# kostas1515/object_detectors

Hardware: AMD Instinct MI355X
Metric: images/sec (fwd+bwd) YOLOv3 640px bs=32 (higher is better)
Workload: dtype bf16; 1 GPU; YOLOv3 Darknet-53 training step (fwd+loss+bwd+SGD step), synthetic COCO 640px, per-GPU bs=32, 7 GT/img, random-init weights; global_batch=32, parallelism=dp1

## Files before the change

### include/mi355det.h

```cpp
#ifndef MI355DET_H
#define MI355DET_H

#include <stddef.h>
#include <stdint.h>

#ifdef __cplusplus
extern "C" {
#endif

#define MI355DET_OK 0
#define MI355DET_EINVAL (-1)
#define MI355DET_ELAUNCH (-2)
#define MI355DET_EWORKSPACE (-3)

#define MI355DET_MAX_SCALES 4
#define MI355DET_MAX_ANCHORS 8

const char* mi355det_last_error(void);
int mi355det_debug_set(int key, int value);
int mi355det_debug_ptr(int key, void* ptr);
int mi355det_version(void);

typedef struct {
  int32_t num_scales, na, num_classes, pad0;
// ... 94 lines not shown
                        float wy, float ww, float wh, float* rois, int64_t* out_labels, int64_t* out_matched, float* out_regression_targets,
                        void* stream);

int mi355det_match_anchors(const float* gt, const float* anchors, int32_t m, int64_t n, float high_thr,
                           float low_thr, int allow_low_quality, uint32_t* gt_best, int64_t* matches,
                           void* stream);

int mi355det_box_encode(const float* reference_boxes, const float* proposals, float* out, int64_t n,
                        float wx, float wy, float ww, float wh, void* stream);
int mi355det_box_decode(const float* codes, const float* boxes, float* out, int64_t n, int32_t k,
                        float wx, float wy, float ww, float wh, float clip, void* stream);

int mi355det_anchor_grid(const float* cell, int32_t a, int32_t gh, int32_t gw, int32_t stride_h,
                         int32_t stride_w, float* out, void* stream);

int mi355det_sigmoid_focal_loss(const float* x, const float* t, const float* scale, const uint8_t* valid,
                                int64_t rows, int32_t k, float alpha, float gamma, float grad_scale,
                                float* loss_sum, float* grad, void* stream);
int mi355det_sigmoid_focal_loss_elem(const float* x, const float* t, int64_t n, float alpha, float gamma, float* loss,
                                     float* grad, void* stream);

int mi355det_retina_cls_loss(const float* logits, const int64_t* matched, const int64_t* gt_labels,
                             const float* scale, int64_t rows, int32_t k, float alpha, float gamma,
                             float grad_scale, float* loss_sum, float* grad, void* stream);

int mi355det_retina_loss(const float* cls_logits, const float* bbox_regression, const float* anchors, const int64_t* matched,
                         const float* gt_boxes, const int64_t* gt_labels, const int32_t* gt_offsets,
                         const float* class_scale, int32_t n_images, int64_t rows_per_image, int32_t k, float alpha,
                         float gamma, float grad_scale, float* num_fg, float* losses, float* grad_logits,
                         float* grad_regression, void* stream);

typedef struct {
  int32_t n_levels;
  int32_t anchors_per_pixel;
  int64_t pixels[8];
  void* grad[8];
  int32_t grad_ld[8];
} mi355det_level_grads;
int mi355det_retina_loss_lv(const float* cls_logits, const float* bbox_regression, const float* anchors, const int64_t* matched,
                            const float* gt_boxes, const int64_t* gt_labels, const int32_t* gt_offsets, const float* class_scale,
                            int32_t n_images, int64_t rows_per_image, int32_t k, float alpha, float gamma, float grad_scale,
                            float* num_fg, float* losses, const mi355det_level_grads* cls_levels, float* grad_regression, void* stream);

int mi355det_roi_align(const float* const* feats, const int32_t* hs, const int32_t* ws, const float* scales,
                       int32_t num_levels, const float* rois, int32_t num_rois, int32_t channels,
                       int32_t pooled_h, int32_t pooled_w, int32_t sampling_ratio, int aligned, int32_t k_min,
                       int32_t k_max, float* out, const float* grad_out, float* const* grad_feats, void* stream);

int mi355det_roi_align_nhwc(const void* const* feats, const int32_t* hs, const int32_t* ws, const int32_t* lds,
                            const float* scales, int32_t num_levels, const float* rois, int32_t num_rois,
                            int32_t channels, int32_t pooled_h, int32_t pooled_w, int32_t sampling_ratio, int aligned,
                            int32_t k_min, int32_t k_max, float* out, const float* grad_out, float* const* grad_feats,
                            void* stream);

int mi355det_topk(const float* x, int32_t rows, int64_t n, int64_t row_stride, int32_t k, float min_value,
                  int64_t* idx_out, float* val_out, int32_t* count_out, void* stream);
size_t mi355det_topk_workspace(int32_t rows);
int mi355det_topk_ws(const float* x, int32_t rows, int64_t n, int64_t row_stride, int32_t k, float min_value, int64_t* idx_out,
                     float* val_out, int32_t* count_out, void* workspace, size_t workspace_bytes, void* stream);

int mi355det_topk_segments(const float* x, int32_t rows, int64_t row_stride, int32_t nseg, const int64_t* seg_start, const int64_t* seg_n,
                           const int32_t* seg_k, float min_value, int64_t* const* idx_out, float* const* val_out, int32_t* const* count_out,
                           void* workspace, size_t workspace_bytes, void* stream);

typedef struct {
  int32_t n, h, w, cin;
  int32_t ho, wo, cout;
  int32_t ksize, stride, pad;
  int32_t in_ld, out_ld;
} mi355det_conv_shape;

int mi355det_conv_fwd(const mi355det_conv_shape* s, const void* x, const void* w, const float* bias,
                      void* y, int out_f32, float* stats, int32_t cout_pad, void* stream);
typedef struct {
  const float* scale;
  const float* shift;
  const void* residual;
  int32_t residual_ld;
  int32_t relu;
  int64_t out_image_stride;
  float slope;
} mi355det_conv_epilogue;
int mi355det_conv_fwd_ex(const mi355det_conv_shape* s, const void* x, const void* w, const mi355det_conv_epilogue* e,
                         void* y, int out_f32, int32_t cout_pad, void* stream);
int mi355det_conv_autotune_mode(int on);

typedef struct {
  uint32_t table;
  int32_t value;
  uint64_t key;
} mi355det_tune_entry;
size_t mi355det_tune_export(void* buf, size_t cap);
int mi355det_tune_import(const void* buf, size_t bytes, int replace);
int mi355det_tune_lock(int on);
int mi355det_tune_clear(void);
int mi355det_conv_stats_rows(const mi355det_conv_shape* s, int32_t cout_pad);
int mi355det_stem_im2col(const float* img, void* out, int32_t n, int32_t h, int32_t w, void* stream);

int mi355det_stem_l1_rows(int32_t n, int32_t h, int32_t w);
int mi355det_stem_l1_fwd(const float* img, const void* w0, const float* scale_shift0, float slope, const void* w1, void* a0,
                         int32_t a0_ld, void* z1, int32_t z1_ld, float* stats, int32_t n, int32_t h, int32_t w, void* stream);
int mi355det_stem_l1_fwd_eval(const float* img, const void* w0, const float* scale_shift0, float slope, const void* w1,
                              const float* scale_shift1, void* a1, int32_t a1_ld, int32_t n, int32_t h, int32_t w, void* stream);
int mi355det_stem_rows(int32_t n, int32_t h, int32_t w);
int mi355det_stem_fwd_stats(const float* img, const void* w, float* partial, int32_t n, int32_t h, int32_t wd, void* stream);
int mi355det_stem_fwd_apply(const float* img, const void* w, const float* scale_shift, float slope, void* a, int32_t a_ld,
                            int32_t n, int32_t h, int32_t wd, void* stream);
int mi355det_stem_bwd_reduce(const float* img, const void* w, const float* scale_shift, float slope, const void* da,
                             int32_t da_ld, float* partial, int32_t n, int32_t h, int32_t wd, void* stream);
int mi355det_stem_bwd_apply_wgrad(const float* img, const void* w, const float* scale_shift, const float* sums, float slope,
                                  const void* da, int32_t da_ld, float* slab, float* dw, float* dgamma, float* dbeta,
                                  int32_t n, int32_t h, int32_t wd, void* stream);

int mi355det_stem_bwd_fused(const float* img, const void* w, const float* scale_shift, float slope, const void* da, int32_t da_ld,
                            float* slab, float* ag, float* sums, int32_t n, int32_t h, int32_t wd, void* stream);
int mi355det_stem_bwd_finish(const void* w, const float* scale_shift, const float* ag, const float* sums, int64_t count, float* dw,
                             float* dgamma, float* dbeta, void* stream);

int mi355det_conv_dgrad(const mi355det_conv_shape* s, const void* dy, const void* wt, void* dx,
                        const void* residual, int32_t residual_ld, void* stream);

int mi355det_conv_dgrad_mask(const mi355det_conv_shape* s, const void* dy, const void* wt, void* dx, const void* act, int32_t act_ld,
                             const float* scale, int32_t relu, void* stream);
size_t mi355det_conv_dgrad_workspace(const mi355det_conv_shape* s);
int mi355det_conv_dgrad_ws(const mi355det_conv_shape* s, const void* dy, const void* wt, void* dx, const void* residual, int32_t residual_ld,
                           void* workspace, size_t workspace_bytes, void* stream);

int mi355det_conv_dgrad_bn_rows(const mi355det_conv_shape* s);
int mi355det_conv_dgrad_bn(const mi355det_conv_shape* s, const void* dy, const void* wt, void* dx, const void* residual,
                           int32_t residual_ld, const void* z, int32_t z_ld, const float* scale_shift, float slope,
                           float* partials, void* stream);
int mi355det_bn_bwd_sum_partials(const float* partials, int32_t rows, int32_t c, int32_t c_pad, float* sums,
                                 void* stream);

size_t mi355det_conv_wgrad_workspace(const mi355det_conv_shape* s);
int mi355det_conv_wgrad_autotune(const mi355det_conv_shape* s, const void* x, const void* dy, float* dw,
                                 void* workspace, size_t workspace_bytes, void* stream);
int mi355det_conv_wgrad(const mi355det_conv_shape* s, const void* x, const void* dy, float* dw,
                        float* dbias, void* workspace, size_t workspace_bytes, void* stream);

size_t mi355det_dgrad_pack_elems(const mi355det_conv_shape* s);
int mi355det_pack_weights(const mi355det_conv_shape* s, const float* w, int w_is_ohwi, void* w_fwd,
                          int32_t cout_pad, void* w_dgrad, void* stream);
typedef struct {
  const float* w;
  void* w_fwd;
  void* w_dgrad;
  mi355det_conv_shape shape;
  int32_t cout_pad, w_is_ohwi;
} mi355det_pack_item;
size_t mi355det_pack_table_bytes(const mi355det_pack_item* items, int32_t n, int32_t* n_entries, int32_t* n_blocks);
int mi355det_pack_table_build(const mi355det_pack_item* items, int32_t n, void* host_table, size_t host_bytes);
int mi355det_pack_weights_batched(const void* dev_table, int32_t n_entries, int32_t n_blocks, void* stream);
int mi355det_unpack_wgrad(const mi355det_conv_shape* s, const float* dw, float* grad, void* stream);

size_t mi355det_gconv_pack_elems(const mi355det_conv_shape* s, int32_t groups);
int mi355det_gconv_pack_weights(const mi355det_conv_shape* s, int32_t groups, const float* w, int w_is_ohwi, void* w_fwd, void* w_dgrad,
                                void* stream);
int mi355det_gconv_fwd_ex(const mi355det_conv_shape* s, int32_t groups, const void* x, const void* w_fwd, const mi355det_conv_epilogue* e,
                          void* y, int out_f32, void* stream);
int mi355det_gconv_dgrad(const mi355det_conv_shape* s, int32_t groups, const void* dy, const void* w_dgrad, void* dx, void* stream);
size_t mi355det_gconv_wgrad_workspace(const mi355det_conv_shape* s, int32_t groups);
int mi355det_gconv_wgrad(const mi355det_conv_shape* s, int32_t groups, const void* x, const void* dy, float* dw, void* workspace,
                         size_t workspace_bytes, void* stream);

int mi355det_bn_finalize(const float* stats, int32_t rows, int32_t c, int32_t c_pad, int64_t count,
                         const float* gamma, const float* beta, float eps, float momentum,
                         float* running_mean, float* running_var,
                         float* scale_shift , void* stream);
int mi355det_bn_fold_partials_f64(const float* stats, int32_t rows, int32_t c, int32_t c_pad, double* sums64, void* stream);
int mi355det_bn_finalize_f64(const double* sums64, int32_t c, int32_t c_pad, int64_t count, const float* gamma, const float* beta,
                             float eps, float momentum, float* running_mean, float* running_var, float* scale_shift,
                             void* stream);
int mi355det_bn_eval_scale_shift(int32_t c, const float* gamma, const float* beta, const float* running_mean,
                                 const float* running_var, float eps, float* scale_shift, void* stream);
int mi355det_add_bf16(const void* a, int32_t a_ld, const void* b, int32_t b_ld, int32_t c, int64_t pixels,
                      void* out, int32_t out_ld, void* stream);
int mi355det_bn_act_fwd(const void* z, int32_t z_ld, const float* scale_shift, int32_t c, int64_t pixels,
                        float slope, const void* residual, int32_t res_ld, void* out, int32_t out_ld,
                        void* stream);
int mi355det_bn_act_bwd_reduce(const void* g1, int32_t g1_ld, const void* g2, int32_t g2_ld, const void* z,
                               int32_t z_ld, const float* scale_shift, int32_t c, int64_t pixels,
                               float slope, float* sums , void* stream);
size_t mi355det_bn_act_bwd_reduce_workspace(int32_t c, int64_t pixels);
int mi355det_bn_act_bwd_reduce_det(const void* g1, int32_t g1_ld, const void* g2, int32_t g2_ld, const void* z,
                                   int32_t z_ld, const float* scale_shift, int32_t c, int64_t pixels,
                                   float slope, float* sums, void* workspace, size_t workspace_bytes, void* stream);
int mi355det_bn_act_bwd_apply(const void* g1, int32_t g1_ld, const void* g2, int32_t g2_ld, const void* z,
                              int32_t z_ld, const float* scale_shift, const float* sums, const float* gamma,
                              int32_t c, int64_t pixels, float slope, void* dz, int32_t dz_ld,
                              float* dgamma, float* dbeta, void* stream);

int mi355det_upsample2x_fwd(const void* x, int32_t x_ld, int32_t n, int32_t h, int32_t w, int32_t c, void* out,
                            int32_t out_ld, void* stream);
int mi355det_upsample2x_bwd(const void* g, int32_t g_ld, int32_t n, int32_t h, int32_t w, int32_t c, void* out,
                            int32_t out_ld, void* stream);

int mi355det_resnet_stem_fwd(const float* img, const float* mean, const float* inv_std, const void* w, const float* scale,
                             const float* shift, int32_t relu, void* out, int32_t out_ld, int32_t n, int32_t h, int32_t wd,
                             void* stream);

int mi355det_im2col_nchw(const float* img, const float* mean, const float* inv_std, void* out, int32_t n, int32_t c,
                         int32_t h, int32_t w, int32_t ksize, int32_t stride, int32_t pad, int32_t kpad, void* stream);
int mi355det_maxpool3x3s2(const void* x, int32_t x_ld, int32_t n, int32_t h, int32_t w, int32_t c, void* out,
                          int32_t out_ld, void* stream);
int mi355det_maxpool3x3s2_bwd(const void* x, int32_t x_ld, const void* g, int32_t g_ld, int32_t n, int32_t h, int32_t w,
                              int32_t c, void* dx, int32_t dx_ld, void* stream);
int mi355det_relu_affine_bwd(const void* g1, int32_t g1_ld, const void* g2, int32_t g2_ld, const void* a, int32_t a_ld,
                             const float* scale, int32_t c, int64_t pixels, int relu, void* dz, int32_t dz_ld,
                             void* gm, int32_t gm_ld, void* stream);
int mi355det_upsample_nearest_add(const void* x, int32_t x_ld, int32_t n, int32_t h, int32_t w, int32_t c,
                                  const void* lateral, int32_t lateral_ld, int32_t out_h, int32_t out_w, void* out,
                                  int32_t out_ld, void* stream);
int mi355det_upsample_nearest_bwd(const void* g, int32_t g_ld, int32_t n, int32_t h, int32_t w, int32_t c, int32_t g_h,
                                  int32_t g_w, const void* accumulate, int32_t accumulate_ld, void* out,
                                  int32_t out_ld, void* stream);
int mi355det_cast_rows_bf16(const float* src, int64_t src_image_stride, int64_t src_row_stride, int32_t n, int64_t rows,
                            int32_t cols, float mul, void* dst, int32_t dst_ld, void* stream);

int mi355det_sgd_step(float* w, float* g, float* momentum_buf, int64_t n, float lr, float momentum, float dampening,
                      float weight_decay, float grad_scale, int nesterov, int first_step, int zero_grad, void* stream);
int mi355det_adam_step(float* w, float* g, float* exp_avg, float* exp_avg_sq, int64_t n, float lr, float beta1,
                       float beta2, float eps, float weight_decay, float grad_scale, int32_t step, int zero_grad,
                       void* stream);
int mi355det_grad_nonfinite(const float* g, int64_t n, int32_t* flag, void* stream);
int mi355det_sgd_step_guarded(float* w, float* g, float* momentum_buf, int64_t n, float lr, float momentum, float dampening,
                              float weight_decay, float grad_scale, int nesterov, int first_step, int zero_grad,
                              const int32_t* skip_flag, void* stream);
int mi355det_adam_step_guarded(float* w, float* g, float* exp_avg, float* exp_avg_sq, int64_t n, float lr, float beta1,
                               float beta2, float eps, float weight_decay, float grad_scale, int32_t step, int zero_grad,
                               const int32_t* skip_flag, void* stream);


size_t mi355det_fastrcnn_loss_workspace(int32_t n);
int mi355det_fastrcnn_loss(const float* class_logits, const float* box_regression, const int64_t* labels,
                           const float* regression_targets, const float* class_scale, const float* class_weights, int32_t n,
                           int32_t k, int32_t loss_type, float* losses, float* grad_logits, float* grad_box, void* workspace,
                           size_t workspace_bytes, void* stream);

int mi355det_resize_bilinear(const float* in, int32_t planes, int32_t c, int32_t h, int32_t w, const float* mean, const float* stdv,
                             float* out, int32_t out_h, int32_t out_w, int32_t pad_h, int32_t pad_w, void* stream);
int mi355det_resize_boxes(const float* boxes, float* out, int64_t n, int32_t orig_h, int32_t orig_w, int32_t new_h, int32_t new_w,
                          void* stream);

#define MI355DET_INGEST_TILE_H 16
#define MI355DET_INGEST_TILE_W 64
typedef struct {
  int64_t offset;
  int32_t h, w;
  int32_t out_h, out_w;
  int32_t flip;
  int32_t first_tile;
} mi355det_ingest_image;
int32_t mi355det_ingest_tiles(int32_t pad_h, int32_t pad_w);
int mi355det_ingest_u8(const uint8_t* packed, int64_t packed_bytes, const mi355det_ingest_image* table,
                       const mi355det_ingest_image* table_dev, int32_t n, const float* mean, const float* stdv, float* out, int32_t pad_h,
                       int32_t pad_w, void* stream);
int mi355det_flip_resize_boxes(const float* boxes, float* out, int64_t g, const int64_t* box_offsets,
                               const mi355det_ingest_image* table_dev, int32_t n, void* stream);

#define MI355DET_PHOTO_MAX_OPS 5
#define MI355DET_PHOTO_BLOCK_PIXELS 4096
#define MI355DET_PHOTO_BRIGHTNESS 1
#define MI355DET_PHOTO_CONTRAST 2
#define MI355DET_PHOTO_SATURATION 3
#define MI355DET_PHOTO_HUE 4
typedef struct {
  int64_t offset;
  int64_t pixels;
  int32_t first_block;
  int32_t n_ops;
  int32_t op[MI355DET_PHOTO_MAX_OPS];
  float factor[MI355DET_PHOTO_MAX_OPS];
  int32_t perm[3];
  int32_t reserved;
} mi355det_photo_image;
typedef struct {
  int64_t offset;
  int32_t h, w;
  int32_t canvas_h, canvas_w;
  int32_t paste_top, paste_left;
  int32_t crop_top, crop_left;
  int32_t crop_h, crop_w;
  int32_t out_h, out_w;
  int32_t flip;
  int32_t first_tile;
  uint32_t fill_rgb;
  int32_t reserved;
} mi355det_ingest_aug_image;
int32_t mi355det_photo_blocks(int64_t pixels);
int mi355det_photometric_u8(uint8_t* packed, int64_t packed_bytes, const mi355det_photo_image* table,
                            const mi355det_photo_image* table_dev, int32_t m, uint64_t* sums, void* stream);
int mi355det_ingest_aug_u8(const uint8_t* packed, int64_t packed_bytes, const mi355det_ingest_aug_image* table,
                           const mi355det_ingest_aug_image* table_dev, int32_t n, const float* mean, const float* stdv, float* out,
                           int32_t pad_h, int32_t pad_w, void* stream);

#define MI355DET_YOLO_TILE_H 16
#define MI355DET_YOLO_TILE_W 64
typedef struct {
  int32_t s;
  int16_t w[4];
} mi355det_cubic_tap;
typedef struct {
  int64_t offset;
  int32_t h, w;
  int32_t channels;
// ... 202 lines not shown
```

### include/mi355det_f16.h

```cpp
#ifndef MI355DET_F16_H
#define MI355DET_F16_H
#include "mi355det.h"
#ifdef __cplusplus
extern "C" {
#endif

int mi355det_conv_autotune_mode_f16(int on);
int mi355det_conv_dgrad_f16(const mi355det_conv_shape* s, const void* dy, const void* wt, void* dx, const void* residual, int32_t residual_ld, void* stream);
int mi355det_conv_dgrad_bn_f16(const mi355det_conv_shape* s, const void* dy, const void* wt, void* dx, const void* residual, int32_t residual_ld, const void* z, int32_t z_ld, const float* scale_shift, float slope, float* partials, void* stream);
int mi355det_conv_dgrad_bn_rows_f16(const mi355det_conv_shape* s);
int mi355det_conv_dgrad_mask_f16(const mi355det_conv_shape* s, const void* dy, const void* wt, void* dx, const void* act, int32_t act_ld, const float* scale, int32_t relu, void* stream);
size_t mi355det_conv_dgrad_workspace_f16(const mi355det_conv_shape* s);
int mi355det_conv_dgrad_ws_f16(const mi355det_conv_shape* s, const void* dy, const void* wt, void* dx, const void* residual, int32_t residual_ld, void* workspace, size_t workspace_bytes, void* stream);
int mi355det_conv_fwd_f16(const mi355det_conv_shape* s, const void* x, const void* w, const float* bias, void* y, int out_f32, float* stats, int32_t cout_pad, void* stream);
int mi355det_conv_fwd_ex_f16(const mi355det_conv_shape* s, const void* x, const void* w, const mi355det_conv_epilogue* e, void* y, int out_f32, int32_t cout_pad, void* stream);
int mi355det_conv_stats_rows_f16(const mi355det_conv_shape* s, int32_t cout_pad);
int mi355det_debug_ptr_f16(int key, void* ptr);
int mi355det_debug_set_f16(int key, int value);
size_t mi355det_dgrad_pack_elems_f16(const mi355det_conv_shape* s);
int mi355det_pack_table_build_f16(const mi355det_pack_item* items, int32_t n, void* host_table, size_t host_bytes);
size_t mi355det_pack_table_bytes_f16(const mi355det_pack_item* items, int32_t n, int32_t* n_entries, int32_t* n_blocks);
int mi355det_pack_weights_f16(const mi355det_conv_shape* s, const float* w, int w_is_ohwi, void* w_fwd, int32_t cout_pad, void* w_dgrad, void* stream);
int mi355det_pack_weights_batched_f16(const void* dev_table, int32_t n_entries, int32_t n_blocks, void* stream);
int mi355det_stem_im2col_f16(const float* img, void* out, int32_t n, int32_t h, int32_t w, void* stream);
int mi355det_unpack_wgrad_f16(const mi355det_conv_shape* s, const float* dw, float* grad, void* stream);
int mi355det_conv_wgrad_f16(const mi355det_conv_shape* s, const void* x, const void* dy, float* dw, float* dbias, void* workspace, size_t workspace_bytes, void* stream);
int mi355det_conv_wgrad_autotune_f16(const mi355det_conv_shape* s, const void* x, const void* dy, float* dw, void* workspace, size_t workspace_bytes, void* stream);
size_t mi355det_conv_wgrad_workspace_f16(const mi355det_conv_shape* s);
int mi355det_add_bf16_f16(const void* a, int32_t a_ld, const void* b, int32_t b_ld, int32_t c, int64_t pixels, void* out, int32_t out_ld, void* stream);
int mi355det_bn_act_bwd_apply_f16(const void* g1, int32_t g1_ld, const void* g2, int32_t g2_ld, const void* z, int32_t z_ld, const float* scale_shift, const float* sums, const float* gamma, int32_t c, int64_t pixels, float slope, void* dz, int32_t dz_ld, float* dgamma, float* dbeta, void* stream);
int mi355det_bn_act_bwd_reduce_f16(const void* g1, int32_t g1_ld, const void* g2, int32_t g2_ld, const void* z, int32_t z_ld, const float* scale_shift, int32_t c, int64_t pixels, float slope, float* sums , void* stream);
int mi355det_bn_act_bwd_reduce_det_f16(const void* g1, int32_t g1_ld, const void* g2, int32_t g2_ld, const void* z, int32_t z_ld, const float* scale_shift, int32_t c, int64_t pixels, float slope, float* sums, void* workspace, size_t workspace_bytes, void* stream);
size_t mi355det_bn_act_bwd_reduce_workspace_f16(int32_t c, int64_t pixels);
int mi355det_bn_act_fwd_f16(const void* z, int32_t z_ld, const float* scale_shift, int32_t c, int64_t pixels, float slope, const void* residual, int32_t res_ld, void* out, int32_t out_ld, void* stream);
int mi355det_nchw_f32_to_nhwc_f16(const float* x, int32_t n, int32_t c, int32_t h, int32_t w, void* out, int out_is_bf16, int32_t out_ld, void* stream);
int mi355det_nhwc_to_nchw_f32_f16(const void* x, int x_is_bf16, int32_t x_ld, int32_t n, int32_t c, int32_t h, int32_t w, float* out, void* stream);
int mi355det_upsample2x_bwd_f16(const void* g, int32_t g_ld, int32_t n, int32_t h, int32_t w, int32_t c, void* out, int32_t out_ld, void* stream);
int mi355det_upsample2x_fwd_f16(const void* x, int32_t x_ld, int32_t n, int32_t h, int32_t w, int32_t c, void* out, int32_t out_ld, void* stream);
int mi355det_stem_bwd_apply_wgrad_f16(const float* img, const void* w, const float* scale_shift, const float* sums, float slope, const void* da, int32_t da_ld, float* slab, float* dw, float* dgamma, float* dbeta, int32_t n, int32_t h, int32_t wd, void* stream);
int mi355det_stem_bwd_finish_f16(const void* w, const float* scale_shift, const float* ag, const float* sums, int64_t count, float* dw, float* dgamma, float* dbeta, void* stream);
int mi355det_stem_bwd_fused_f16(const float* img, const void* w, const float* scale_shift, float slope, const void* da, int32_t da_ld, float* slab, float* ag, float* sums, int32_t n, int32_t h, int32_t wd, void* stream);
int mi355det_stem_bwd_reduce_f16(const float* img, const void* w, const float* scale_shift, float slope, const void* da, int32_t da_ld, float* partial, int32_t n, int32_t h, int32_t wd, void* stream);
int mi355det_stem_fwd_apply_f16(const float* img, const void* w, const float* scale_shift, float slope, void* a, int32_t a_ld, int32_t n, int32_t h, int32_t wd, void* stream);
int mi355det_stem_fwd_stats_f16(const float* img, const void* w, float* partial, int32_t n, int32_t h, int32_t wd, void* stream);
int mi355det_stem_rows_f16(int32_t n, int32_t h, int32_t w);
int mi355det_stem_l1_fwd_f16(const float* img, const void* w0, const float* scale_shift0, float slope, const void* w1, void* a0, int32_t a0_ld, void* z1, int32_t z1_ld, float* stats, int32_t n, int32_t h, int32_t w, void* stream);
int mi355det_stem_l1_fwd_eval_f16(const float* img, const void* w0, const float* scale_shift0, float slope, const void* w1, const float* scale_shift1, void* a1, int32_t a1_ld, int32_t n, int32_t h, int32_t w, void* stream);
int mi355det_stem_l1_rows_f16(int32_t n, int32_t h, int32_t w);

#ifdef __cplusplus
}
#endif
#endif
```

### object_detectors_amd/_lib.py

```python
import ctypes as C
import os

HERE = os.path.dirname(os.path.abspath(__file__))
LIB_PATH = os.environ.get("MI355DET_LIB", os.path.join(HERE, "libmi355det.so"))

MAX_SCALES, MAX_ANCHORS = 4, 8

vp, i32, i64, f32, sz = C.c_void_p, C.c_int32, C.c_int64, C.c_float, C.c_size_t


class YoloGeom(C.Structure):
    _fields_ = [("num_scales", i32), ("na", i32), ("num_classes", i32), ("pad0", i32),
                ("img_size", f32), ("ignore_thr", f32), ("iou_type", i32), ("pad1", i32),
                ("grid", i32 * MAX_SCALES), ("off", i32 * (MAX_SCALES + 1)),
                ("anchor_w", (f32 * MAX_ANCHORS) * MAX_SCALES), ("anchor_h", (f32 * MAX_ANCHORS) * MAX_SCALES)]


class HeadView(C.Structure):
    _fields_ = [("ptr", vp), ("sb", i64), ("sc", i64), ("sp", i64)]


class YoloLossCfg(C.Structure):
    _fields_ = [("lambda_iou", f32), ("lambda_xy", f32), ("lambda_wh", f32), ("lambda_conf", f32),
                ("lambda_no_conf", f32), ("lambda_cls", f32), ("alpha", f32), ("gamma", f32),
                ("grad_scale", f32), ("grad_is_bf16", i32), ("class_weights", vp), ("class_loss", i32), ("reduction_mean", i32),
                ("eq_mask", vp)]


class ConvShape(C.Structure):
    _fields_ = [("n", i32), ("h", i32), ("w", i32), ("cin", i32), ("ho", i32), ("wo", i32), ("cout", i32),
                ("ksize", i32), ("stride", i32), ("pad", i32), ("in_ld", i32), ("out_ld", i32)]


class ConvEpilogue(C.Structure):
    _fields_ = [("scale", vp), ("shift", vp), ("residual", vp), ("residual_ld", i32), ("relu", i32), ("out_image_stride", i64),
                ("slope", C.c_float)]


class LevelGrads(C.Structure):
    _fields_ = [("n_levels", i32), ("anchors_per_pixel", i32), ("pixels", i64 * 8), ("grad", vp * 8), ("grad_ld", i32 * 8)]


MASK_MAX_IMAGES = 64


class MaskImages(C.Structure):
    _fields_ = [("masks", vp * MASK_MAX_IMAGES), ("h", i32 * MASK_MAX_IMAGES), ("w", i32 * MASK_MAX_IMAGES), ("n_images", i32)]


INGEST_TILE_H, INGEST_TILE_W = 16, 64


class IngestImage(C.Structure):
    _fields_ = [("offset", i64), ("h", i32), ("w", i32), ("out_h", i32), ("out_w", i32), ("flip", i32), ("first_tile", i32)]


PHOTO_MAX_OPS, PHOTO_BLOCK_PIXELS = 5, 4096
PHOTO_OPS = {"brightness": 1, "contrast": 2, "saturation": 3, "hue": 4}


class PhotoImage(C.Structure):
    _fields_ = [("offset", i64), ("pixels", i64), ("first_block", i32), ("n_ops", i32), ("op", i32 * PHOTO_MAX_OPS),
                ("factor", f32 * PHOTO_MAX_OPS), ("perm", i32 * 3), ("reserved", i32)]


class IngestAugImage(C.Structure):
    _fields_ = [("offset", i64), ("h", i32), ("w", i32), ("canvas_h", i32), ("canvas_w", i32), ("paste_top", i32), ("paste_left", i32),
                ("crop_top", i32), ("crop_left", i32), ("crop_h", i32), ("crop_w", i32), ("out_h", i32), ("out_w", i32), ("flip", i32),
                ("first_tile", i32), ("fill_rgb", C.c_uint32), ("reserved", i32)]


YOLO_TILE_H, YOLO_TILE_W = 16, 64


class CubicTap(C.Structure):
    _fields_ = [("s", i32), ("w", C.c_int16 * 4)]


class YoloImage(C.Structure):
    _fields_ = [("offset", i64), ("h", i32), ("w", i32), ("channels", i32), ("flip", i32), ("xtab", i32), ("ytab", i32)]


class PackItem(C.Structure):
    _fields_ = [("w", vp), ("w_fwd", vp), ("w_dgrad", vp), ("shape", ConvShape), ("cout_pad", i32), ("w_is_ohwi", i32)]


P = C.POINTER
PROTOTYPES = {
    "mi355det_last_error": (C.c_char_p, []),
    "mi355det_version": (C.c_int, []),
    "mi355det_debug_set": (C.c_int, [C.c_int, C.c_int]),
    "mi355det_debug_ptr": (C.c_int, [C.c_int, vp]),
    "mi355det_bbox_iou": (C.c_int, [vp, vp, vp, i64, i64, C.c_int, C.c_int, C.c_int, vp]),
    "mi355det_yolo_assign": (C.c_int, [P(YoloGeom), vp, vp, i32, i32, i32, vp, vp, vp, vp, vp]),
    "mi355det_yolo_loss_workspace": (sz, [i32, i64]),
    "mi355det_yolo_loss": (C.c_int, [P(YoloGeom), P(YoloLossCfg), P(HeadView), P(HeadView), vp, vp, vp, vp, vp, vp,
                                      i32, i32, vp, sz, vp, vp]),
    "mi355det_yolo_decode": (C.c_int, [P(YoloGeom), P(HeadView), vp, i32, C.c_int, vp, vp, vp, vp]),
    "mi355det_yolo_candidates_workspace": (sz, [i32, i64]),
    "mi355det_yolo_candidates": (C.c_int, [vp, vp, vp, i32, i64, i32, f32, vp, vp, i32, vp, sz, vp]),
    "mi355det_nms_workspace": (sz, [i32, i32]),
    "mi355det_nms_majority": (C.c_int, [vp, vp, i32, i32, f32, i32, vp, vp, vp, vp, sz, vp]),
    "mi355det_box_iou": (C.c_int, [vp, vp, vp, i64, i64, vp]),
    "mi355det_nms": (C.c_int, [vp, vp, vp, i32, f32, vp, vp, vp, sz, vp]),
    "mi355det_nms_batch": (C.c_int, [vp, vp, vp, i32, i32, C.c_float, vp, vp, vp, sz, vp]),
    "mi355det_topk_segments": (C.c_int, [vp, i32, i64, i32, vp, vp, vp, f32, vp, vp, vp, vp, sz, vp]),
    "mi355det_rpn_proposals_workspace": (sz, [i32, vp, i32, i32]),
    "mi355det_rpn_proposals": (C.c_int, [vp, vp, vp, vp, i32, vp, i32, i32, i32, f32, f32, f32, f32, vp, vp, vp, vp, sz, vp]),
    "mi355det_retina_detections_workspace": (sz, [i32, vp, i32, i32, i32]),
    "mi355det_retina_detections": (C.c_int, [vp, vp, vp, vp, i32, i32, i32, vp, f32, i32, f32, i32, f32, vp, vp, vp, vp, vp, sz, vp]),
    "mi355det_roi_detections_workspace": (sz, [i32, i32, i32, i32]),
    "mi355det_roi_detections": (C.c_int, [vp, vp, vp, vp, i32, i32, i32, f32, i32, f32, f32, f32, f32, f32, f32, f32, i32, vp, vp, vp, vp, vp, vp, sz, vp]),
    "mi355det_rpn_loss": (C.c_int, [vp, vp, vp, vp, i64, vp, i32, vp, i32, vp, vp, vp, vp]),
    "mi355det_roi_match": (C.c_int, [vp, vp, i32, i32, vp, vp, vp, f32, f32, i32, vp, vp, vp, vp]),
    "mi355det_roi_sample": (C.c_int, [vp, vp, i32, i32, vp, vp, i32, vp, vp, vp, vp, vp, vp, f32, f32, f32, f32, vp, vp, vp, vp, vp]),
    "mi355det_match_anchors": (C.c_int, [vp, vp, i32, i64, f32, f32, C.c_int, vp, vp, vp]),
    "mi355det_box_encode": (C.c_int, [vp, vp, vp, i64, f32, f32, f32, f32, vp]),
    "mi355det_box_decode": (C.c_int, [vp, vp, vp, i64, i32, f32, f32, f32, f32, f32, vp]),
    "mi355det_anchor_grid": (C.c_int, [vp, i32, i32, i32, i32, i32, vp, vp]),
    "mi355det_sigmoid_focal_loss": (C.c_int, [vp, vp, vp, vp, i64, i32, f32, f32, f32, vp, vp, vp]),
    "mi355det_sigmoid_focal_loss_elem": (C.c_int, [vp, vp, i64, f32, f32, vp, vp, vp]),
    "mi355det_retina_cls_loss": (C.c_int, [vp, vp, vp, vp, i64, i32, f32, f32, f32, vp, vp, vp]),
    "mi355det_roi_align_nhwc": (C.c_int, [vp, vp, vp, vp, vp, i32, vp, i32, i32, i32, i32, i32, C.c_int, i32, i32, vp, vp, vp, vp]),
    "mi355det_roi_align": (C.c_int, [vp, vp, vp, vp, i32, vp, i32, i32, i32, i32, i32, C.c_int, i32, i32, vp, vp, vp, vp]),
    "mi355det_topk": (C.c_int, [vp, i32, i64, i64, i32, f32, vp, vp, vp, vp]),
    "mi355det_conv_fwd": (C.c_int, [P(ConvShape), vp, vp, vp, vp, C.c_int, vp, i32, vp]),
    "mi355det_conv_dgrad": (C.c_int, [P(ConvShape), vp, vp, vp, vp, i32, vp]),
    "mi355det_conv_dgrad_mask": (C.c_int, [P(ConvShape), vp, vp, vp, vp, i32, vp, i32, vp]),
    "mi355det_conv_dgrad_workspace": (sz, [P(ConvShape)]),
    "mi355det_conv_dgrad_ws": (C.c_int, [P(ConvShape), vp, vp, vp, vp, i32, vp, sz, vp]),
    "mi355det_conv_wgrad_workspace": (sz, [P(ConvShape)]),
    "mi355det_conv_wgrad_autotune": (C.c_int, [P(ConvShape), vp, vp, vp, vp, sz, vp]),
    "mi355det_conv_wgrad": (C.c_int, [P(ConvShape), vp, vp, vp, vp, vp, sz, vp]),
    "mi355det_dgrad_pack_elems": (sz, [P(ConvShape)]),
    "mi355det_pack_weights": (C.c_int, [P(ConvShape), vp, C.c_int, vp, i32, vp, vp]),
    "mi355det_pack_table_bytes": (sz, [P(PackItem), i32, P(i32), P(i32)]),
    "mi355det_pack_table_build": (C.c_int, [P(PackItem), i32, vp, sz]),
    "mi355det_pack_weights_batched": (C.c_int, [vp, i32, i32, vp]),
    "mi355det_unpack_wgrad": (C.c_int, [P(ConvShape), vp, vp, vp]),
    "mi355det_gconv_pack_elems": (sz, [P(ConvShape), i32]),
    "mi355det_gconv_pack_weights": (C.c_int, [P(ConvShape), i32, vp, C.c_int, vp, vp, vp]),
    "mi355det_gconv_fwd_ex": (C.c_int, [P(ConvShape), i32, vp, vp, P(ConvEpilogue), vp, C.c_int, vp]),
    "mi355det_gconv_dgrad": (C.c_int, [P(ConvShape), i32, vp, vp, vp, vp]),
    "mi355det_gconv_wgrad_workspace": (sz, [P(ConvShape), i32]),
    "mi355det_gconv_wgrad": (C.c_int, [P(ConvShape), i32, vp, vp, vp, vp, sz, vp]),
    "mi355det_conv_autotune_mode": (C.c_int, [C.c_int]),
    "mi355det_tune_export": (sz, [vp, sz]),
    "mi355det_tune_import": (C.c_int, [vp, sz, C.c_int]),
    "mi355det_tune_lock": (C.c_int, [C.c_int]),
    "mi355det_tune_clear": (C.c_int, []),
    "mi355det_conv_stats_rows": (C.c_int, [P(ConvShape), i32]),
    "mi355det_stem_im2col": (C.c_int, [vp, vp, i32, i32, i32, vp]),
    "mi355det_stem_rows": (C.c_int, [i32, i32, i32]),
    "mi355det_stem_l1_rows": (C.c_int, [i32, i32, i32]),
    "mi355det_stem_l1_fwd": (C.c_int, [vp, vp, vp, f32, vp, vp, i32, vp, i32, vp, i32, i32, i32, vp]),
    "mi355det_stem_l1_fwd_eval": (C.c_int, [vp, vp, vp, f32, vp, vp, vp, i32, i32, i32, i32, vp]),
    "mi355det_stem_fwd_stats": (C.c_int, [vp, vp, vp, i32, i32, i32, vp]),
    "mi355det_stem_fwd_apply": (C.c_int, [vp, vp, vp, f32, vp, i32, i32, i32, i32, vp]),
    "mi355det_stem_bwd_reduce": (C.c_int, [vp, vp, vp, f32, vp, i32, vp, i32, i32, i32, vp]),
    "mi355det_stem_bwd_apply_wgrad": (C.c_int, [vp, vp, vp, vp, f32, vp, i32, vp, vp, vp, vp, i32, i32, i32, vp]),
    "mi355det_stem_bwd_fused": (C.c_int, [vp, vp, vp, f32, vp, i32, vp, vp, vp, i32, i32, i32, vp]),
    "mi355det_stem_bwd_finish": (C.c_int, [vp, vp, vp, vp, i64, vp, vp, vp, vp]),
    "mi355det_bn_finalize": (C.c_int, [vp, i32, i32, i32, i64, vp, vp, f32, f32, vp, vp, vp, vp]),
    "mi355det_bn_eval_scale_shift": (C.c_int, [i32, vp, vp, vp, vp, f32, vp, vp]),
    "mi355det_bn_fold_partials_f64": (C.c_int, [vp, i32, i32, i32, vp, vp]),
    "mi355det_bn_finalize_f64": (C.c_int, [vp, i32, i32, i64, vp, vp, f32, f32, vp, vp, vp, vp]),
    "mi355det_conv_dgrad_bn_rows": (C.c_int, [P(ConvShape)]),
    "mi355det_conv_dgrad_bn": (C.c_int, [P(ConvShape), vp, vp, vp, vp, i32, vp, i32, vp, C.c_float, vp, vp]),
    "mi355det_bn_bwd_sum_partials": (C.c_int, [vp, i32, i32, i32, vp, vp]),
    "mi355det_conv_fwd_ex": (C.c_int, [P(ConvShape), vp, vp, P(ConvEpilogue), vp, C.c_int, i32, vp]),
    "mi355det_retina_loss": (C.c_int, [vp] * 8 + [i32, i64, i32, C.c_float, C.c_float, C.c_float, vp, vp, vp, vp, vp]),
    "mi355det_retina_loss_lv": (C.c_int, [vp] * 8 + [i32, i64, i32, C.c_float, C.c_float, C.c_float, vp, vp, P(LevelGrads), vp, vp]),
    "mi355det_im2col_nchw": (C.c_int, [vp, vp, vp, vp] + [i32] * 8 + [vp]),
    "mi355det_maxpool3x3s2": (C.c_int, [vp, i32, i32, i32, i32, i32, vp, i32, vp]),
    "mi355det_resnet_stem_fwd": (C.c_int, [vp, vp, vp, vp, vp, vp, i32, vp, i32, i32, i32, i32, vp]),
    "mi355det_maxpool3x3s2_bwd": (C.c_int, [vp, i32, vp, i32, i32, i32, i32, i32, vp, i32, vp]),
    "mi355det_relu_affine_bwd": (C.c_int, [vp, i32, vp, i32, vp, i32, vp, i32, i64, C.c_int, vp, i32, vp, i32, vp]),
    "mi355det_upsample_nearest_add": (C.c_int, [vp, i32, i32, i32, i32, i32, vp, i32, i32, i32, vp, i32, vp]),
    "mi355det_upsample_nearest_bwd": (C.c_int, [vp, i32, i32, i32, i32, i32, i32, i32, vp, i32, vp, i32, vp]),
    "mi355det_cast_rows_bf16": (C.c_int, [vp, i64, i64, i32, i64, i32, C.c_float, vp, i32, vp]),
    "mi355det_sgd_step": (C.c_int, [vp, vp, vp, i64] + [C.c_float] * 5 + [C.c_int] * 3 + [vp]),
    "mi355det_adam_step": (C.c_int, [vp, vp, vp, vp, i64] + [C.c_float] * 6 + [i32, C.c_int, vp]),
    "mi355det_sgd_step_guarded": (C.c_int, [vp, vp, vp, i64] + [C.c_float] * 5 + [C.c_int] * 3 + [vp, vp]),
    "mi355det_adam_step_guarded": (C.c_int, [vp, vp, vp, vp, i64] + [C.c_float] * 6 + [i32, C.c_int, vp, vp]),
    "mi355det_grad_nonfinite": (C.c_int, [vp, i64, vp, vp]),
    "mi355det_add_bf16": (C.c_int, [vp, i32, vp, i32, i32, i64, vp, i32, vp]),
    "mi355det_bn_act_fwd": (C.c_int, [vp, i32, vp, i32, i64, f32, vp, i32, vp, i32, vp]),
    "mi355det_bn_act_bwd_reduce": (C.c_int, [vp, i32, vp, i32, vp, i32, vp, i32, i64, f32, vp, vp]),
    "mi355det_bn_act_bwd_reduce_workspace": (sz, [i32, i64]),
    "mi355det_bn_act_bwd_reduce_det": (C.c_int, [vp, i32, vp, i32, vp, i32, vp, i32, i64, f32, vp, vp, sz, vp]),
    "mi355det_bn_act_bwd_apply": (C.c_int, [vp, i32, vp, i32, vp, i32, vp, vp, vp, i32, i64, f32, vp, i32, vp, vp, vp]),
    "mi355det_upsample2x_fwd": (C.c_int, [vp, i32, i32, i32, i32, i32, vp, i32, vp]),
    "mi355det_upsample2x_bwd": (C.c_int, [vp, i32, i32, i32, i32, i32, vp, i32, vp]),
    "mi355det_nchw_f32_to_nhwc": (C.c_int, [vp, i32, i32, i32, i32, vp, C.c_int, i32, vp]),
    "mi355det_nhwc_to_nchw_f32": (C.c_int, [vp, C.c_int, i32, i32, i32, i32, i32, vp, vp]),
    "mi355det_topk_workspace": (sz, [i32]),
    "mi355det_topk_ws": (C.c_int, [vp, i32, i64, i64, i32, C.c_float, vp, vp, vp, vp, sz, vp]),
    "mi355det_resize_bilinear": (C.c_int, [vp, i32, i32, i32, i32, vp, vp, vp, i32, i32, i32, i32, vp]),
    "mi355det_resize_boxes": (C.c_int, [vp, vp, i64, i32, i32, i32, i32, vp]),
    "mi355det_ingest_tiles": (i32, [i32, i32]),
    "mi355det_ingest_u8": (C.c_int, [vp, i64, vp, vp, i32, vp, vp, vp, i32, i32, vp]),
    "mi355det_flip_resize_boxes": (C.c_int, [vp, vp, i64, vp, vp, i32, vp]),
    "mi355det_photo_blocks": (i32, [i64]),
    "mi355det_photometric_u8": (C.c_int, [vp, i64, vp, vp, i32, vp, vp]),
    "mi355det_ingest_aug_u8": (C.c_int, [vp, i64, vp, vp, i32, vp, vp, vp, i32, i32, vp]),
    "mi355det_yolo_ingest_u8": (C.c_int, [vp, i64, vp, vp, i32, vp, i64, vp, vp, i32, vp]),
    "mi355det_yolo_targets": (C.c_int, [vp, vp, i64, vp, vp, i32, vp, vp, vp]),
    "mi355det_coco_rows": (C.c_int, [vp, i32, vp, vp, i32, i64, f32, f32, f32, i32, i32, vp, vp, vp, vp]),
    "mi355det_fastrcnn_loss_workspace": (sz, [i32]),
    "mi355det_fastrcnn_loss": (C.c_int, [vp, vp, vp, vp, vp, vp, i32, i32, i32, vp, vp, vp, vp, sz, vp]),
    "mi355det_mask_roi_pool": (C.c_int, [vp, vp, vp, vp, vp, i32, vp, i32, i32, i32, i32, i32, i32, i32, vp, i32, vp, i32, vp, vp]),
    "mi355det_mask_targets": (C.c_int, [P(MaskImages), vp, vp, i32, i32, vp, vp]),
    "mi355det_mask_loss_workspace": (sz, [i32]),
    "mi355det_mask_loss": (C.c_int, [vp, i32, vp, vp, vp, vp, i32, i32, i32, vp, vp, vp, vp, vp, vp, sz, vp]),
    "mi355det_mask_probs": (C.c_int, [vp, i32, vp, vp, vp, i32, i32, vp, vp]),
    "mi355det_mask_resize_nearest": (C.c_int, [vp, i32, i32, i32, vp, i32, i32, vp]),
    "mi355det_mask_flip_resize_nearest": (C.c_int, [vp, i32, i32, i32, vp, i32, i32, i32, vp]),
    "mi355det_paste_masks": (C.c_int, [vp, vp, i32, i32, i32, i32, i32, vp, vp]),
    "mi355det_mask_rle_workspace": (sz, [i32, i32]),
    "mi355det_mask_rle_count": (C.c_int, [vp, vp, vp, i32, i32, i32, i32, i32, f32, vp, vp, sz, vp]),
    "mi355det_mask_rle_emit": (C.c_int, [vp, vp, vp, i32, i32, i32, i32, i32, f32, vp, i64, vp, i64, vp, vp, vp, sz, vp]),
    "mi355det_flip_resize_keypoints": (C.c_int, [vp, vp, i64, i32, vp, vp, vp, i32, vp]),
    "mi355det_keypoint_targets": (C.c_int, [vp, vp, i32, vp, vp, i32, i32, i32, i32, vp, vp, vp, vp]),
    "mi355det_keypoint_heatmaps": (C.c_int, [vp, i32, i32, i32, i32, vp, vp]),
    "mi355det_keypoint_loss_workspace": (sz, [i32, i32]),
    "mi355det_keypoint_loss": (C.c_int, [vp, i32, i32, i32, i32, vp, vp, vp, vp, vp, vp, vp, vp, sz, vp]),
    "mi355det_heatmaps_to_keypoints": (C.c_int, [vp, vp, i32, i32, i32, vp, vp, vp]),
    "mi355det_rle_to_string": (i64, [vp, i64, C.c_char_p, i64]),
    "mi355det_rle_from_string": (i64, [C.c_char_p, vp, i64]),
    "mi355det_rle_strings_count": (C.c_int, [vp, i64, vp, vp, vp, i64, vp, vp, vp, vp]),
    "mi355det_rle_strings_emit": (C.c_int, [vp, i64, vp, vp, i64, vp, i64, vp, i64, vp, vp, vp]),
    "mi355det_rle_boundary_plan": (i64, [vp, i64, i64, vp, vp, i64, i64, vp, vp, vp]),
    "mi355det_rle_boundary_count": (C.c_int, [vp, i64, vp, vp, i64, vp, vp, vp, vp, vp, vp, i64, i64, i64, vp, vp, sz, vp]),
    "mi355det_rle_boundary_emit": (C.c_int, [vp, i64, vp, vp, i64, vp, vp, vp, vp, vp, vp, i64, i64, i64, vp, i64, vp, i64, vp, vp, vp, sz, vp]),
    "mi355det_poly_points_count": (C.c_int, [vp, vp, vp, vp, i32, i32, vp, vp]),
    "mi355det_poly_points_emit": (C.c_int, [vp, vp, vp, vp, i32, i32, vp, i64, vp, i64, vp]),
    "mi355det_poly_events": (C.c_int, [vp, vp, vp, vp, vp, i32, i32, vp, i64, vp, vp]),
    "mi355det_poly_runs_count": (C.c_int, [vp, vp, vp, vp, vp, vp, i32, i32, vp, vp]),
    "mi355det_poly_runs_emit": (C.c_int, [vp, vp, vp, vp, vp, vp, i32, i32, vp, i64, vp, i64, vp, vp, vp]),
    "mi355det_rle_decode": (C.c_int, [vp, vp, i32, i32, i32, vp, vp]),
    "mi355det_coco_iou": (C.c_int, [i32, i64, vp, vp, vp, i64, i64, i64, vp, vp, vp, vp, vp, vp, i64, i64, vp, vp, vp, i64, i64, vp, vp, vp, vp]),
    "mi355det_coco_match": (C.c_int, [i64, vp, vp, vp, i64, i64, i64, vp, vp, vp, vp, vp, i32, vp, i32, vp, vp, vp, vp, vp]),
    "mi355det_lvis_match": (C.c_int, [i64, vp, vp, vp, i64, i64, i64, vp, vp, vp, vp, vp, vp, i32, vp, i32, vp, vp, vp, vp, vp]),
    "mi355det_coco_oks": (C.c_int, [i64, vp, vp, vp, i64, i64, i64, i32, vp, vp, vp, vp, vp, vp, vp]),
    "mi355det_keypoints_match": (C.c_int, [i64, vp, vp, vp, i64, i64, i64, vp, vp, vp, vp, vp, vp, i32, vp, i32, vp, vp, vp, vp, vp]),
    "mi355det_coco_accumulate": (C.c_int, [i32, vp, vp, i64, i64, vp, vp, vp, vp, vp, vp, i32, i32, vp, i32, vp, i32, vp, vp, vp, vp]),
    "mi355det_coco_bootstrap": (C.c_int, [i32, vp, vp, i64, i64, vp, vp, vp, vp, vp, i32, i32, vp, i32, vp, i32, vp, vp, vp, i32, i32, vp, vp, vp]),
    "mi355det_category_frequencies_workspace": (sz, [i32, i32]),
    "mi355det_category_frequencies_lds_categories": (C.c_int, []),
    "mi355det_category_frequencies": (C.c_int, [vp, vp, i64, i32, i32, vp, vp, vp, vp, sz, vp]),
    "mi355det_idf_table": (C.c_int, [vp, vp, i32, i64, vp, vp]),
    "mi355det_kmeans_limit": (C.c_int, [C.c_int]),
    "mi355det_box_features": (C.c_int, [vp, vp, vp, i64, i32, vp, vp, vp, vp]),
    "mi355det_kmeans_workspace": (sz, [i64, i32, i32, i32, i32]),
    "mi355det_kmeans_check": (C.c_int, [vp, vp, i64, i32, i32, i32, vp, vp]),
    "mi355det_kmeans_begin": (C.c_int, [i64, i32, i32, i32, i32, vp, vp, vp, sz, vp]),
    "mi355det_kmeans_passes": (C.c_int, [vp, vp, i64, i32, i32, i32, i32, i32, i32, i32, vp, vp, vp, vp, vp, vp, vp, vp, sz, vp]),
    "mi355det_kmeans_assign": (C.c_int, [vp, vp, i64, i32, i32, i32, i32, vp, vp, vp, vp]),
    "mi355det_box_disagreement": (C.c_int, [i64, vp, i64, vp, vp, vp, i64, vp, vp, vp, i64, vp, vp, C.c_double, vp, vp, vp, vp]),
    "mi355det_tide_classify": (C.c_int, [i64, vp, vp, i64, vp, vp, i64, vp, vp, vp, vp, vp, vp, vp, C.c_double, C.c_double, vp, vp, vp, vp, vp, vp]),
    "mi355det_tide_fixes": (C.c_int, [i64, vp, vp, i64, vp, vp, i64, vp, vp, vp, vp, vp, vp, vp, vp, vp, vp, vp, vp, vp, vp, vp, vp]),
    "mi355det_wbf_lds_clusters": (C.c_int, []),
    "mi355det_wbf_fuse": (C.c_int, [vp, i64, i64, vp, vp, C.c_double, i32, C.c_double, C.c_double, vp, vp, vp, vp, vp, vp, vp]),
    "mi355det_pooled_tile": (C.c_int, []),
    "mi355det_pooled_accumulate_workspace": (sz, [i64, i32, i32, i32]),
    "mi355det_pooled_accumulate": (C.c_int, [vp, i64, vp, vp, i32, vp, i64, vp, vp, vp, i32, i32, vp, i32, vp, vp, vp, vp, sz, vp]),
}

def _f16_twins():
    import re
    txt = open(os.path.join(HERE, "csrc", "f16_names.h")).read().split("// ---- cross-file symbols")[0]
    return re.findall(r"#define (mi355det_[a-z0-9_]+) \1_f16", txt)


F16_TWINS = _f16_twins()
for _n in F16_TWINS:
    PROTOTYPES[_n + "_f16"] = PROTOTYPES[_n]

_lib = None


class Mi355detError(RuntimeError):
    pass


def lib():
    global _lib
    if _lib is None:
        if not os.path.exists(LIB_PATH):
            raise Mi355detError(
                f"{LIB_PATH} not found: build it with `python -m object_detectors_amd.build` "
# ... 58 lines not shown
```

### object_detectors_amd/csrc/conv_kernels.hip

```cpp
#include "common.h"

#include <cstdlib>

#include <unordered_map>

#include "tune_record.h"
#include "tune_timing.h"

using namespace mi355;

#include "igemm_common.h"

extern int g_wgrad_general;
extern int g_wgrad_force_dbg;
extern int g_wgrad8_off;
extern int g_wgrad_ablate;
extern int g_dgrad_s2_off;
extern int g_conv_strict;
int mi355det_internal_dgrad_s2(const mi355det_conv_shape* s, const void* dy, const void* wt, void* dx, const void* residual, int32_t residual_ld,
                               void* stream, int probe = 0);

namespace {

#define STAMP(v) do { if (PROF) { __builtin_amdgcn_sched_barrier(0); asm volatile("s_memtime %0\n\ts_waitcnt lgkmcnt(0)" : "=s"(v) :: "memory"); __builtin_amdgcn_sched_barrier(0); } } while (0)

template <int WM, int WN, int TM, int TN, int BK, int NST, int EPI, bool PROF = false, bool ILV = false, int OCC = 0, int ABL = 0>
__global__ __launch_bounds__(WM* WN * 64, (OCC > 0 ? OCC : (WM * WN >= 8 ? 2 : 1))) void igemm_kernel(const IgemmParams p) {
  unsigned long long t_a = 0, t_b = 0, t_c = 0, t_d = 0, t_e = 0, c_wait = 0, c_bar = 0, c_issue = 0, c_comp = 0, t_begin = 0, t_loop = 0;
  STAMP(t_begin);
  constexpr int NT = WM * WN * 64;
  constexpr int NW = WM * WN;
  constexpr int BM = WM * TM * 16, BN = WN * TN * 16;
  constexpr int ROWB = BK * 2;
  constexpr int R = 1024 / ROWB;
  constexpr int CPR = BK / 8;
  constexpr int A_INSTR = BM / R, B_INSTR = BN / R;
  constexpr int A_PER = (A_INSTR + NW - 1) / NW, B_PER = (B_INSTR + NW - 1) / NW;
  constexpr int PER = A_PER + B_PER;
  constexpr int STAGE = (BM + BN) * ROWB;
  constexpr int D = NST - 1;
  static_assert(A_INSTR % NW == 0, "A tile must split evenly over the waves");
  extern __shared__ __attribute__((aligned(16))) char smem[];
  int* s_toff = (int*)(smem + NST * STAGE);

  const int tid = threadIdx.x, lane = tid & 63;
  const int wid = __builtin_amdgcn_readfirstlane(tid >> 6);
  const int wm = wid % WM, wn = wid / WM;

  const int ntn = p.CoutPad / BN;
  int nblk = gridDim.x;
  int bid = blockIdx.x;
  int sp = 0;
  if (p.ksplit > 1) {
    const int q = __builtin_amdgcn_readfirstlane(bid / p.ksplit);
    sp = bid - q * p.ksplit;
    bid = q;
    nblk = __builtin_amdgcn_readfirstlane(nblk / p.ksplit);
  }
  {
    const int q = nblk / 8, r = nblk % 8, xcd = bid % 8, loc = bid / 8;
    bid = (xcd < r ? xcd * (q + 1) : r * (q + 1) + (xcd - r) * q) + loc;
  }
  const int mt = bid / ntn, nt = bid - mt * ntn;
  const int m0 = mt * BM, n0 = nt * BN;

  if (tid == 0) {
#pragma unroll
    for (int t = 0; t < MAX_TAPS; ++t)
      if (t < p.T) s_toff[t] = ((p.dy[t] * p.Win + p.dx[t]) * p.ldin + p.tap_pad) * 2;
  }

  unsigned long long t_p1 = 0, t_p2 = 0, t_p3 = 0, t_p4 = 0;
  STAMP(t_p1);
  const int n_first = (int)fdiv(fdiv((unsigned)m0, p.dMW), p.dMH);
  const int Ktot = p.T * p.Cin;
  const srd_t rsrc_x = make_srd(p.x + (long long)n_first * p.Hin * p.Win * p.ldin - p.tap_pad, 0x7FFFFFF0u);
  const srd_t rsrc_w = make_srd(p.w + (long long)n0 * Ktot, 0x7FFFFFF0u);

  const int lrow = lane / CPR, cpos = lane % CPR;
  int a_voff[A_PER];
  unsigned a_valid[A_PER];
#pragma unroll
  for (int i = 0; i < A_PER; ++i) {
    const int instr = wid * A_PER + i;
    const int row = instr * R + lrow;
    const int m = m0 + row;
    unsigned vm = 0;
    int voff = OOB_VOFF;
    if (p.lin_in) {
      if (m < p.M) {
        voff = ((m - n_first * p.Hin * p.Win) * p.ldin + (cpos ^ swz<BK>(row)) * 8) * 2;
        vm = 1u;
      }
    } else if (m < p.M) {
      const int t1 = (int)fdiv((unsigned)m, p.dMW), xx = m - t1 * p.MW;
      const int n = (int)fdiv((unsigned)t1, p.dMH), yy = t1 - n * p.MH;
      const int iy0 = yy * p.sin, ix0 = xx * p.sin;
      voff = ((((n - n_first) * p.Hin + iy0) * p.Win + ix0) * p.ldin + (cpos ^ swz<BK>(row)) * 8) * 2;
#pragma unroll
      for (int t = 0; t < MAX_TAPS; ++t) {
        if (t >= p.T) break;
        const int dyt = (int)((p.dy_pack >> (4 * t)) & 0xF) - 2, dxt = (int)((p.dx_pack >> (4 * t)) & 0xF) - 2;
        const bool ok = (unsigned)(iy0 + dyt) < (unsigned)p.Hin && (unsigned)(ix0 + dxt) < (unsigned)p.Win;
        vm |= ok ? (1u << t) : 0u;
      }
    }
    a_voff[i] = voff;
    a_valid[i] = vm;
  }
  if (PROF) asm volatile("s_nop 0" ::"v"(a_voff[0]), "v"(a_valid[A_PER - 1]));
  STAMP(t_p2);
  int b_voff[B_PER], b_instr[B_PER];
#pragma unroll
  for (int i = 0; i < B_PER; ++i) {
    const int instr = (wid * B_PER + i) % B_INSTR;
    const int row = instr * R + lrow;
    b_instr[i] = instr;
    b_voff[i] = (row * Ktot + (cpos ^ swz<BK>(row)) * 8) * 2;
  }
  __builtin_amdgcn_s_waitcnt(0xC07F);
  STAMP(t_p3);
  __builtin_amdgcn_s_barrier();
  STAMP(t_p4);

  const int cin_steps = __builtin_amdgcn_readfirstlane((p.ksplit > 1 ? p.Cin / p.ksplit : p.Cin) / BK);
  const int c0b = sp * cin_steps * (BK * 2);
  const int ksteps = ABL == 5 ? 0 : p.T * cin_steps;
  int pf_t = 0, pf_c = 0;

  auto stage = [&](int s, int buf) {
    const int coff = c0b + pf_c * (BK * 2);
    const int soff = __builtin_amdgcn_readfirstlane(s_toff[pf_t]) + coff;
    const int boff = pf_t * (p.Cin * 2) + coff;
    char* sa = smem + buf * STAGE;
    char* sb = sa + BM * ROWB;
#pragma unroll
    for (int i = 0; i < A_PER; ++i) {
      const int instr = wid * A_PER + i;
      bufld16(rsrc_x, sa + instr * 1024, ((a_valid[i] >> pf_t) & 1u) ? a_voff[i] : OOB_VOFF, soff);
    }
#pragma unroll
    for (int i = 0; i < B_PER; ++i) bufld16(rsrc_w, sb + b_instr[i] * 1024, b_voff[i], boff);
    if (++pf_c == cin_steps) {
      pf_c = 0;
      ++pf_t;
    }
  };

  auto issue_piece = [&](int q, int boff, int soff, int tap, int buf) {
    char* sa = smem + buf * STAGE;
    char* sb = sa + BM * ROWB;
    if (q < A_PER) {
      const int instr = wid * A_PER + q;
      bufld16(rsrc_x, sa + instr * 1024, ((a_valid[q] >> tap) & 1u) ? a_voff[q] : OOB_VOFF, soff);
    } else {
      bufld16(rsrc_w, sb + b_instr[q - A_PER] * 1024, b_voff[q - A_PER], boff);
    }
// ... 921 lines not shown
  return 0;
}

int mi355det_conv_stats_rows(const mi355det_conv_shape* s, int32_t cout_pad) {
  (void)cout_pad;
  return s ? (int)(((long long)s->n * s->ho * s->wo + 127) / 128) : 0;
}

static int conv_fwd_impl(const mi355det_conv_shape* s, const void* x, const void* w, const float* bias, void* y, int out_f32, float* stats,
                         int32_t cout_pad, const mi355det_conv_epilogue* ex, void* stream) {
  if (int e = check_shape(s, "conv_fwd")) return e;
  if (int e = ensure_zero_page()) return e;
  if (cout_pad < s->cout) return fail(MI355DET_EINVAL, "%s: cout_pad < cout", "conv_fwd");
  if (!out_f32 && (s->cout % 8)) return fail(MI355DET_EINVAL, "%s: 16-bit outputs need cout %% 8 == 0 (got %lld)", "conv_fwd", s->cout);
  IgemmParams p{};
  p.x = (const bf16_t*)x;
  p.w = (const bf16_t*)w;
  p.y = y;
  p.bias = bias;
  p.stats = stats;
  p.zero = g_zero_page;
  p.MH = s->ho;
  p.MW = s->wo;
  p.M = s->n * s->ho * s->wo;
  p.Hin = s->h; p.Win = s->w; p.ldin = s->in_ld; p.Cin = s->cin; p.sin = s->stride;
  p.Hout = s->ho; p.Wout = s->wo; p.ldout = s->out_ld; p.so = 1; p.oy0 = 0; p.ox0 = 0;
  p.Cout = s->cout; p.CoutPad = cout_pad;
  p.T = s->ksize * s->ksize;
  for (int kh = 0; kh < s->ksize; ++kh)
    for (int kw = 0; kw < s->ksize; ++kw) {
      p.dy[kh * s->ksize + kw] = kh - s->pad;
      p.dx[kh * s->ksize + kw] = kw - s->pad;
    }
  p.dMW = make_fastdiv((unsigned)p.MW);
  p.dMH = make_fastdiv((unsigned)p.MH);
  p.ynstride = (long long)s->ho * s->wo * s->out_ld;
  set_tap_pad(p);
  if (ex) {
    p.scale = ex->scale;
    p.bias = ex->shift;
    p.relu = ex->relu;
    p.slope = ex->slope;
    p.res = (const bf16_t*)ex->residual;
    p.ldres = ex->residual_ld;
    if (ex->out_image_stride) {
      if (!out_f32) return fail(MI355DET_EINVAL, "%s: out_image_stride needs an fp32 output", "conv_fwd_ex");
      p.ynstride = ex->out_image_stride;
    }
    if (out_f32 && ex->residual) return fail(MI355DET_EINVAL, "%s: residual needs a bf16 output", "conv_fwd_ex");
    const int r = out_f32 ? dispatch_igemm<EPI_F32>(p, S(stream)) : dispatch_igemm<EPI_AFF>(p, S(stream));
    return r < 0 ? r : 0;
  }
  const int r = out_f32 ? dispatch_igemm<EPI_F32>(p, S(stream)) : stats ? dispatch_igemm<EPI_STATS>(p, S(stream)) : dispatch_igemm<EPI_PLAIN>(p, S(stream));
  return r < 0 ? r : 0;
}

int mi355det_conv_fwd(const mi355det_conv_shape* s, const void* x, const void* w, const float* bias, void* y, int out_f32, float* stats,
                      int32_t cout_pad, void* stream) {
  return conv_fwd_impl(s, x, w, bias, y, out_f32, stats, cout_pad, nullptr, stream);
}

int mi355det_conv_fwd_ex(const mi355det_conv_shape* s, const void* x, const void* w, const mi355det_conv_epilogue* e, void* y, int out_f32,
                         int32_t cout_pad, void* stream) {
  if (!e) return fail(MI355DET_EINVAL, "%s: null epilogue", "conv_fwd_ex");
  return conv_fwd_impl(s, x, w, nullptr, y, out_f32, nullptr, cout_pad, e, stream);
}

static int dgrad_taps(const mi355det_conv_shape* s, int py, int px, int* fwd_tap, int* dy, int* dx) {
  int n = 0;
  const int k = s->ksize, pd = s->pad;
  for (int kh = 0; kh < k; ++kh)
    for (int kw = 0; kw < k; ++kw) {
      if (s->stride == 1) {
        fwd_tap[n] = kh * k + kw;
        dy[n] = pd - kh;
        dx[n] = pd - kw;
        ++n;
      } else {
        const int ny = py + pd - kh, nx = px + pd - kw;
        if ((ny & 1) || (nx & 1)) continue;
        fwd_tap[n] = kh * k + kw;
        dy[n] = ny / 2;
        dx[n] = nx / 2;
        ++n;
      }
    }
  return n;
}

static IgemmParams dgrad_params(const mi355det_conv_shape* s, int py, int px, const void* dy, const void* w, void* dx) {
  IgemmParams p{};
  int ft[9];
  p.T = dgrad_taps(s, py, px, ft, p.dy, p.dx);
  p.x = (const bf16_t*)dy;
  p.w = (const bf16_t*)w;
  p.y = dx;
  p.zero = g_zero_page;
  if (s->stride == 1) {
    p.MH = s->h; p.MW = s->w; p.so = 1;
  } else {
    p.MH = (s->h + 1) / 2; p.MW = (s->w + 1) / 2; p.so = 2; p.oy0 = py; p.ox0 = px;
  }
  p.M = s->n * p.MH * p.MW;
  p.Hin = s->ho; p.Win = s->wo; p.ldin = s->out_ld; p.Cin = s->cout; p.sin = 1;
  p.Hout = s->h; p.Wout = s->w; p.ldout = s->in_ld;
  p.Cout = s->cin; p.CoutPad = (s->cin + 31) / 32 * 32;
  p.dMW = make_fastdiv((unsigned)p.MW);
  p.dMH = make_fastdiv((unsigned)p.MH);
  set_tap_pad(p);
  return p;
}

size_t mi355det_dgrad_pack_elems(const mi355det_conv_shape* s) {
  if (!s) return 0;
  mi355det_conv_shape d = *s;
  d.in_ld = d.cin;
  return dgrad_class_elems(s) + s2cat_elems(&d) + 64;
}

int mi355det_pack_weights(const mi355det_conv_shape* s, const float* w, int w_is_ohwi, void* w_fwd, int32_t cout_pad, void* w_dgrad,
                          void* stream) {
  if (int e = check_shape(s, "pack_weights")) return e;
  const int kk = s->ksize * s->ksize;
  const long long s_co = (long long)s->cin * kk, s_ci = w_is_ohwi ? 1 : kk, s_t = w_is_ohwi ? s->cin : 1;
  if (w_fwd) {
    const long long total = (long long)cout_pad * kk * s->cin;
    hipLaunchKernelGGL(pack_fwd_kernel, dim3((int)min((long long)2048, (total + 255) / 256)), dim3(256), 0, S(stream), w, (bf16_t*)w_fwd, s->cout,
                       cout_pad, s->cin, s->cin, kk, s_co, s_ci, s_t);
  }
  if (w_dgrad) {
    const int cin_pad = (s->cin + 31) / 32 * 32;
    bf16_t* out = (bf16_t*)w_dgrad;
    const int classes = s->stride == 1 ? 1 : 4;
    for (int c = 0; c < classes; ++c) {
      int ft[9] = {0}, dy[9], dx[9];
      const int nt = dgrad_taps(s, c >> 1, c & 1, ft, dy, dx);
      const long long total = (long long)cin_pad * nt * s->cout;
      if (total == 0) continue;
      hipLaunchKernelGGL(pack_dgrad_kernel, dim3((int)min((long long)2048, (total + 255) / 256)), dim3(256), 0, S(stream), w, out, s->cout, s->cin,
                         cin_pad, kk, nt, s_co, s_ci, s_t, ft[0], ft[1], ft[2], ft[3], ft[4], ft[5], ft[6], ft[7], ft[8]);
      out += total;
    }
    mi355det_conv_shape d = *s;
    d.in_ld = d.cin;
    if (s2cat_eligible(&d)) {
      const long long total = (long long)12 * s->cin * s->cout;
      hipLaunchKernelGGL(pack_s2cat_kernel, dim3((int)min((long long)2048, (total + 255) / 256)), dim3(256), 0, S(stream), w,
                         (bf16_t*)w_dgrad + dgrad_class_elems(s), s->cout, s->cin, s_co, s_ci, s_t);
    }
  }
  return check_launch("pack_weights");
}

struct PackEntry {
  const float* src;
  bf16_t* dst;
  long long s_co, s_ci, s_t;
  int total, rows_valid, cin, kk, ntaps, mode, cdim, cob;
  int taps[9];
  int ncib, ncob, pad1;
};
#define PACK_CHUNK 4096

__global__ __launch_bounds__(256) void pack_batched_kernel(const PackEntry* __restrict__ entries, const int2* __restrict__ blocks) {
  const int2 bt = blocks[blockIdx.x];
  const PackEntry e = entries[bt.x];
  if (e.mode == 2) {
    const long long n0 = (long long)2 * e.cin * 2 * e.cdim;
    const int end = min(e.total, bt.y + PACK_CHUNK);
    for (int i = bt.y + threadIdx.x; i < end; i += 256) {
      const int py = i >= n0;
      const long long j = py ? i - n0 : i;
      const int T = py ? 4 : 2;
      const int co = (int)(j % e.cdim), tap = (int)((j / e.cdim) % T), r = (int)(j / ((long long)e.cdim * T));
      const int px = r / e.cin, ci = r - px * e.cin;
      const int oy = py ? tap >> 1 : 0, ox = py ? tap & 1 : tap;
      const int kh = s2cat_k(py, oy), kw = s2cat_k(px, ox);
      float v = 0.f;
      if (kh >= 0 && kw >= 0) v = e.src[co * e.s_co + ci * e.s_ci + (kh * 3 + kw) * e.s_t];
      e.dst[i] = f2s(v);
    }
    return;
  }
  if (e.mode == 0) {
    const int end = min(e.total, bt.y + PACK_CHUNK);
    for (int i = bt.y + threadIdx.x; i < end; i += 256) {
      const int c = i % e.cin, t = (i / e.cin) % e.kk, co = i / (e.cin * e.kk);
      float v = 0.f;
      if (co < e.rows_valid) v = e.src[co * e.s_co + c * e.s_ci + t * e.s_t];
      e.dst[i] = f2s(v);
    }
    return;
  }
  __shared__ float tl[64][33];
  int t = bt.y;
  const int co_blk = t % e.ncob;
  t /= e.ncob;
  const int ci_blk = t % e.ncib, j = t / e.ncib;
  int tap = e.taps[0];
#pragma unroll
  for (int q = 1; q < 9; ++q)
    if (j == q) tap = e.taps[q];
  const int cl = threadIdx.x & 31;
  for (int r = threadIdx.x >> 5; r < e.cob; r += 8) {
    const int co = co_blk * e.cob + r, ci = ci_blk * 32 + cl;
    tl[r][cl] = ci < e.rows_valid ? e.src[co * e.s_co + ci * e.s_ci + tap * e.s_t] : 0.f;
  }
  __syncthreads();
  const int col = threadIdx.x % e.cob;
  for (int r = threadIdx.x / e.cob; r < 32; r += 256 / e.cob) {
    const long long ci = ci_blk * 32 + r;
    e.dst[(ci * e.ntaps + j) * e.cdim + co_blk * e.cob + col] = f2s(tl[col][r]);
  }
}

size_t mi355det_pack_table_bytes(const mi355det_pack_item* items, int32_t n, int32_t* n_entries, int32_t* n_blocks) {
  int ne = 0;
  long long nb = 0;
  for (int i = 0; i < n; ++i) {
    const mi355det_conv_shape* s = &items[i].shape;
    const int kk = s->ksize * s->ksize;
    if (items[i].w_fwd) {
      ++ne;
      nb += ((long long)items[i].cout_pad * kk * s->cin + PACK_CHUNK - 1) / PACK_CHUNK;
    }
    if (items[i].w_dgrad) {
      const int cin_pad = (s->cin + 31) / 32 * 32;
      const int classes = s->stride == 1 ? 1 : 4;
      for (int c = 0; c < classes; ++c) {
        int ft[9], dy[9], dx[9];
        const int nt = dgrad_taps(s, c >> 1, c & 1, ft, dy, dx);
        ++ne;
        const int cob = s->cout % 64 == 0 ? 64 : 32;
        nb += (long long)nt * (cin_pad / 32) * (s->cout / cob);
      }
      mi355det_conv_shape d = *s;
      d.in_ld = d.cin;
      if (s2cat_eligible(&d)) {
        ++ne;
        nb += ((long long)s2cat_elems(&d) + PACK_CHUNK - 1) / PACK_CHUNK;
      }
    }
  }
  if (n_entries) *n_entries = ne;
  if (n_blocks) *n_blocks = (int)nb;
  return (size_t)ne * sizeof(PackEntry) + (size_t)nb * sizeof(int2);
}

int mi355det_pack_table_build(const mi355det_pack_item* items, int32_t n, void* host_table, size_t host_bytes) {
  int ne = 0, nb = 0;
  const size_t need = mi355det_pack_table_bytes(items, n, &ne, &nb);
  if (host_bytes < need) return fail(MI355DET_EWORKSPACE, "%s: host table too small", "pack_table_build");
  PackEntry* E = (PackEntry*)host_table;
  int2* B = (int2*)((char*)host_table + (size_t)ne * sizeof(PackEntry));
  int ei = 0, bi = 0;
  auto add_blocks = [&](int entry, long long total) {
    for (long long o = 0; o < total; o += PACK_CHUNK) B[bi++] = make_int2(entry, (int)o);
  };
  for (int i = 0; i < n; ++i) {
    const mi355det_conv_shape* s = &items[i].shape;
    if (int e = check_shape(s, "pack_table_build")) return e;
    if (items[i].w_dgrad && s->cout % 32 != 0) return fail(MI355DET_EINVAL, "%s: dgrad pack needs cout %% 32 == 0", "pack_table_build");
    const int kk = s->ksize * s->ksize;
    const long long s_co = (long long)s->cin * kk, s_ci = items[i].w_is_ohwi ? 1 : kk, s_t = items[i].w_is_ohwi ? s->cin : 1;
    if (items[i].w_fwd) {
      PackEntry& e = E[ei];
      e = PackEntry{};
      e.src = items[i].w; e.dst = (bf16_t*)items[i].w_fwd; e.s_co = s_co; e.s_ci = s_ci; e.s_t = s_t;
      e.total = items[i].cout_pad * kk * s->cin; e.rows_valid = s->cout; e.cin = s->cin; e.kk = kk; e.mode = 0;
      add_blocks(ei++, e.total);
    }
    if (items[i].w_dgrad) {
      const int cin_pad = (s->cin + 31) / 32 * 32;
      bf16_t* out = (bf16_t*)items[i].w_dgrad;
      const int classes = s->stride == 1 ? 1 : 4;
      for (int c = 0; c < classes; ++c) {
        int ft[9] = {0}, dy[9], dx[9];
        const int nt = dgrad_taps(s, c >> 1, c & 1, ft, dy, dx);
        PackEntry& e = E[ei];
        e = PackEntry{};
        e.src = items[i].w; e.dst = out; e.s_co = s_co; e.s_ci = s_ci; e.s_t = s_t;
        e.total = cin_pad * nt * s->cout; e.rows_valid = s->cin; e.cin = s->cin; e.kk = kk; e.ntaps = nt; e.mode = 1; e.cdim = s->cout;
        for (int q = 0; q < 9; ++q) e.taps[q] = ft[q];
        e.cob = s->cout % 64 == 0 ? 64 : 32;
        e.ncib = cin_pad / 32;
        e.ncob = s->cout / e.cob;
        for (int tix = 0; tix < nt * e.ncib * e.ncob; ++tix) B[bi++] = make_int2(ei, tix);
        ++ei;
        out += e.total;
      }
      mi355det_conv_shape d = *s;
      d.in_ld = d.cin;
      if (s2cat_eligible(&d)) {
        PackEntry& e = E[ei];
        e = PackEntry{};
        e.src = items[i].w; e.dst = (bf16_t*)items[i].w_dgrad + dgrad_class_elems(s); e.s_co = s_co; e.s_ci = s_ci; e.s_t = s_t;
        e.total = (int)s2cat_elems(&d); e.cin = s->cin; e.cdim = s->cout; e.mode = 2;
        add_blocks(ei++, e.total);
      }
    }
  }
  return 0;
}

int mi355det_pack_weights_batched(const void* dev_table, int32_t n_entries, int32_t n_blocks, void* stream) {
  if (!dev_table || n_entries <= 0 || n_blocks <= 0) return fail(MI355DET_EINVAL, "%s: bad table", "pack_weights_batched");
  const PackEntry* E = (const PackEntry*)dev_table;
  const int2* B = (const int2*)((const char*)dev_table + (size_t)n_entries * sizeof(PackEntry));
  hipLaunchKernelGGL(pack_batched_kernel, dim3(n_blocks), dim3(256), 0, S(stream), E, B);
  return check_launch("pack_weights_batched");
}

int mi355det_unpack_wgrad(const mi355det_conv_shape* s, const float* dw, float* grad, void* stream) {
  if (int e = check_shape(s, "unpack_wgrad")) return e;
  const int kk = s->ksize * s->ksize;
  const long long total = (long long)s->cout * s->cin * kk;
  hipLaunchKernelGGL(unpack_wgrad_kernel, dim3((int)min((long long)2048, (total + 255) / 256)), dim3(256), 0, S(stream), dw, grad, s->cout, s->cin,
                     s->cin, kk);
  return check_launch("unpack_wgrad");
}

static int conv_dgrad_impl(const mi355det_conv_shape* s, const void* dy, const void* wt, void* dx, const void* residual, int32_t residual_ld,
                           const void* z, int32_t z_ld, const float* scale_shift, float slope, float* partials, void* stream) {
  if (int e = check_shape(s, "conv_dgrad")) return e;
  if (int e = ensure_zero_page()) return e;
  if (s->cout % 32 != 0) return fail(MI355DET_EINVAL, "%s: Cout (the dgrad reduction dim) must be a multiple of 32 (got %lld)", "conv_dgrad", s->cout);
  if (s->cin % 8 != 0) return fail(MI355DET_EINVAL, "%s: cin must be a multiple of 8 (the epilogue stores 8-channel pieces; got %lld)", "conv_dgrad", s->cin);
  if (!partials && !g_autotune_mode) {
    if (strict_forced() && mi355det_internal_dgrad_s2(s, dy, wt, dx, residual, residual_ld, stream, 1))
      return strict_reject(g_tune, "the shape takes the single-launch stride-2 data gradient");
    const int r = mi355det_internal_dgrad_s2(s, dy, wt, dx, residual, residual_ld, stream);
    if (r != 0) return r < 0 ? r : 0;
  }
  const int cin_pad = (s->cin + 31) / 32 * 32;
  const bf16_t* wp = (const bf16_t*)wt;
  const int classes = s->stride == 1 ? 1 : 4;
  if (!partials && s2cat_eligible(s) && (!residual || residual_ld == s->cin)) {
    const unsigned long long key = ((((unsigned long long)s->n * 4099 + s->h) * 4099 + s->w) * 4099 + s->cin) * 4099 + s->cout + (residual ? 1ull << 62 : 0) + (MI355_F16 ? 1ull << 61 : 0);
    int choice = -1;
    auto it = g_s2cat_tuned.find(key);
    if (it != g_s2cat_tuned.end()) choice = it->second;
    if (g_s2cat_force >= 0) choice = g_s2cat_force;
    auto run_cat = [&]() -> int {
      const bf16_t* wc = (const bf16_t*)wt + dgrad_class_elems(s);
      for (int py = 0; py < 2; ++py) {
        IgemmParams p = dgrad_params(s, py, 0, dy, wc, dx);
        p.T = py ? 4 : 2;
        for (int t = 0; t < p.T; ++t) {
          p.dy[t] = py ? t >> 1 : 0;
          p.dx[t] = py ? t & 1 : t;
        }
        p.res = (const bf16_t*)residual;
        p.ldres = 2 * s->cin;
        p.Wout = s->wo; p.ldout = 2 * s->cin; p.sox = 1;
        p.Cout = 2 * s->cin; p.CoutPad = 2 * s->cin;
        set_tap_pad(p);
        const int e = residual ? dispatch_igemm<EPI_RES>(p, S(stream)) : dispatch_igemm<EPI_PLAIN>(p, S(stream));
        if (e < 0) return e;
        wc += (size_t)2 * s->cin * p.T * s->cout;
      }
      return 0;
    };
    if (g_autotune_mode && g_s2cat_force < 0 && !tune_locked_has(TUNE_S2CAT, key)) {
      EventPair ev;
      if (!ev.ok) return fail(MI355DET_ELAUNCH, "%s: event create failed", "conv_dgrad");
      hipEvent_t e0 = ev.e0, e1 = ev.e1;
      float ms[2] = {0.f, 0.f};
      for (int form = 0; form < 2; ++form) {
        g_s2cat_force = form;
        int e = conv_dgrad_impl(s, dy, wt, dx, residual, residual_ld, nullptr, 0, nullptr, 0.f, nullptr, stream);
        g_autotune_mode = false;
        if (!e) ms[form] = time_candidate([&] { return conv_dgrad_impl(s, dy, wt, dx, residual, residual_ld, nullptr, 0, nullptr, 0.f, nullptr, stream); }, e0, e1, S(stream), &e);
        g_autotune_mode = true;
        g_s2cat_force = -1;
        if (e) return e;
      }
      choice = ms[1] < ms[0] ? 1 : 0;
      g_s2cat_tuned[key] = choice;
      tune_mark_timed(TUNE_S2CAT, key);
      static const bool tune_log = getenv("MI355DET_TUNE_LOG") != nullptr;
      if (tune_log) fprintf(stderr, "[mi355det] stride-2 dgrad %d->%d @%dx%d: four classes %.1f us, concatenated %.1f us\n", s->cin, s->cout, s->h, s->w,
                            ms[0] * 1e3f / 3.f, ms[1] * 1e3f / 3.f);
      if (choice == 1) return run_cat();
    } else if (choice == 1) {
      return run_cat();
    }
  }
  for (int c = 0; c < classes; ++c) {
    IgemmParams p = dgrad_params(s, c >> 1, c & 1, dy, wp, dx);
    if (p.T == 0 && partials) return fail(MI355DET_EINVAL, "%s: 1x1 stride-2 layers are not supported by the fused BN reduction", "conv_dgrad_bn");
    if (p.T == 0) {
      const int mh = (s->h + 1) / 2, mw = (s->w + 1) / 2;
      const long long total = (long long)s->n * mh * mw * (s->cin / 8);
      hipLaunchKernelGGL(lattice_fill_kernel, dim3((int)min((long long)4096, (total + 255) / 256)), dim3(256), 0, S(stream), (bf16_t*)dx, s->in_ld,
                         (const bf16_t*)residual, residual_ld, s->n, s->h, s->w, mh, mw, c >> 1, c & 1, s->cin);
      continue;
    }
    p.res = (const bf16_t*)residual;
    p.ldres = residual_ld;
    int e;
    if (partials) {
      p.z = (const bf16_t*)z;
      p.ldz = z_ld;
      p.ss = scale_shift;
      p.slope = slope;
      p.stats = partials + (long long)c * ((p.M + 127) / 128) * 2 * cin_pad;
      e = dispatch_igemm<EPI_BNRED>(p, S(stream));
    } else {
      e = residual ? dispatch_igemm<EPI_RES>(p, S(stream)) : dispatch_igemm<EPI_PLAIN>(p, S(stream));
    }
    if (e < 0) return e;
    wp += (long long)cin_pad * p.T * s->cout;
  }
  return 0;
}

int mi355det_conv_dgrad(const mi355det_conv_shape* s, const void* dy, const void* wt, void* dx, const void* residual, int32_t residual_ld,
                        void* stream) {
  return conv_dgrad_impl(s, dy, wt, dx, residual, residual_ld, nullptr, 0, nullptr, 0.f, nullptr, stream);
}

int mi355det_conv_dgrad_mask(const mi355det_conv_shape* s, const void* dy, const void* wt, void* dx, const void* act, int32_t act_ld,
                             const float* scale, int32_t relu, void* stream) {
  if (int e = check_shape(s, "conv_dgrad_mask")) return e;
  if (int e = ensure_zero_page()) return e;
  if (!dy || !wt || !dx || !act) return fail(MI355DET_EINVAL, "%s: null argument", "conv_dgrad_mask");
  if (s->stride != 1) return fail(MI355DET_EINVAL, "%s: stride-1 convolutions only", "conv_dgrad_mask");
  if (s->cout % 32 != 0) return fail(MI355DET_EINVAL, "%s: Cout (the dgrad reduction dim) must be a multiple of 32 (got %lld)", "conv_dgrad_mask", s->cout);
  if (s->cin % 8 != 0 || act_ld % 8 != 0 || act_ld < s->cin) return fail(MI355DET_EINVAL, "%s: cin and the activation pitch must be multiples of 8", "conv_dgrad_mask");
  IgemmParams p = dgrad_params(s, 0, 0, dy, wt, dx);
  p.res = (const bf16_t*)act;
  p.ldres = act_ld;
  p.scale = scale;
  p.relu = relu ? 3 : 4;
  const int e = dispatch_igemm<EPI_RES>(p, S(stream));
  return e < 0 ? e : 0;
}

static int dgrad_ksplit(const mi355det_conv_shape* s) {
  if (!s || s->stride != 1 || s->ksize * s->ksize > MAX_TAPS) return 0;
  const int cin_pad = (s->cin + 31) / 32 * 32;
  if (cin_pad % 128 != 0 || s->cout % 64 != 0 || s->in_ld % 8 != 0) return 0;
  const long long M = (long long)s->n * s->h * s->w, K = (long long)s->ksize * s->ksize * s->cout;
  const long long tiles = (M + 127) / 128 * (cin_pad / 128);
  if (tiles > 96 || K < 8192) return 0;
  const int chunks = s->cout / 64;
  int best = 0;
  for (int d = 2; d <= chunks; ++d)
    if (chunks % d == 0 && tiles * d <= 512 && chunks / d >= 4) best = d;
  return best;
}

__global__ __launch_bounds__(256) void splitk_reduce_kernel(const float* __restrict__ part, int S, long long sstride, bf16_t* __restrict__ dx, int ld,
                                                            const bf16_t* __restrict__ res, int ldres, long long M, int C, int CP) {
  const int c8 = C / 8;
  const long long total = M * c8;
  for (long long i = blockIdx.x * 256ll + threadIdx.x; i < total; i += (long long)gridDim.x * 256) {
    const long long m = i / c8;
    const int c = (int)(i - m * c8) * 8;
    float a[8] = {0.f, 0.f, 0.f, 0.f, 0.f, 0.f, 0.f, 0.f};
    const float* src = part + m * CP + c;
    for (int sp = 0; sp < S; ++sp) {
      const float4 v0 = *(const float4*)(src + sp * sstride), v1 = *(const float4*)(src + sp * sstride + 4);
// ... 78 lines not shown
```

### object_detectors_amd/csrc/elem_kernels.hip

```cpp
#include "common.h"

#include <cstdlib>

using namespace mi355;

namespace {

__device__ __forceinline__ void add8(f32x8& a, const f32x8& b) {
#pragma unroll
  for (int k = 0; k < 8; ++k) a.v[k] += b.v[k];
}


template <typename T>
__device__ __forceinline__ void bn_fold_rows(const float* __restrict__ partial, int r0, int r1, int c_pad, int ch, bool load, T& s1, T& s2) {
  __shared__ T sh[8][32][2];
  const int cl = threadIdx.x & 31, rl = threadIdx.x >> 5;
  s1 = 0;
  s2 = 0;
  if (load)
    for (int r = r0 + rl; r < r1; r += 8) {
      s1 += (T)partial[(size_t)r * 2 * c_pad + ch];
      s2 += (T)partial[(size_t)r * 2 * c_pad + c_pad + ch];
    }
  sh[rl][cl][0] = s1;
  sh[rl][cl][1] = s2;
  __syncthreads();
  if (rl == 0)
    for (int r = 1; r < 8; ++r) {
      s1 += sh[r][cl][0];
      s2 += sh[r][cl][1];
    }
}

__device__ __forceinline__ void bn_finalize_channel(double s1, double s2, double count, int ch, int c, const float* __restrict__ gamma,
                                                    const float* __restrict__ beta, float eps, float momentum, float* __restrict__ rmean,
                                                    float* __restrict__ rvar, float* __restrict__ ss) {
  const double mean = s1 / count;
  double var = s2 / count - mean * mean;
  if (var < 0) var = 0;
  const float invstd = (float)(1.0 / sqrt(var + (double)eps));
  const float sc = gamma[ch] * invstd;
  ss[ch] = sc;
  ss[c + ch] = beta[ch] - (float)mean * sc;
  ss[2 * c + ch] = (float)mean;
  ss[3 * c + ch] = invstd;
  if (rmean) {
    rmean[ch] = (1.f - momentum) * rmean[ch] + momentum * (float)mean;
    const double unb = count > 1 ? var * count / (count - 1) : var;
    rvar[ch] = (1.f - momentum) * rvar[ch] + momentum * (float)unb;
  }
}

__device__ __forceinline__ f32x8 bn_act8(const f32x8& z, const float (&sc)[8], const float (&sh)[8], float slope) {
  f32x8 a;
#pragma unroll
  for (int k = 0; k < 8; ++k) {
    const float y = z.v[k] * sc[k] + sh[k];
    a.v[k] = y > 0.f ? y : y * slope;
  }
  return a;
}
__device__ __forceinline__ f32x8 bn_dy8(const f32x8& g, const f32x8& z, const float (&sc)[8], const float (&sh)[8], float slope) {
  f32x8 dy;
#pragma unroll
  for (int k = 0; k < 8; ++k) {
    const float y = z.v[k] * sc[k] + sh[k];
    dy.v[k] = y > 0.f ? g.v[k] : g.v[k] * slope;
  }
  return dy;
}
__device__ __forceinline__ float bn_xhat(float z, float mu, float is) { return (z - mu) * is; }
__device__ __forceinline__ f32x8 bn_dz8(const f32x8& dy, const f32x8& z, const float (&sc)[8], const float (&mu)[8], const float (&is)[8],
                                        const float (&m1)[8], const float (&m2)[8]) {
  f32x8 dz;
#pragma unroll
  for (int k = 0; k < 8; ++k) dz.v[k] = sc[k] * (dy.v[k] - m1[k] - bn_xhat(z.v[k], mu[k], is[k]) * m2[k]);
  return dz;
}

__global__ __launch_bounds__(256) void bn_finalize_kernel(const float* __restrict__ partial, int rows, int c, int c_pad, double count,
                                                          const float* __restrict__ gamma, const float* __restrict__ beta, float eps,
                                                          float momentum, float* __restrict__ rmean, float* __restrict__ rvar,
                                                          float* __restrict__ ss) {
  const int ch = blockIdx.x * 32 + (threadIdx.x & 31);
  double s1, s2;
  bn_fold_rows<double>(partial, 0, rows, c_pad, ch, ch < c, s1, s2);
  if (threadIdx.x < 32 && ch < c) bn_finalize_channel(s1, s2, count, ch, c, gamma, beta, eps, momentum, rmean, rvar, ss);
}

__global__ __launch_bounds__(1024) void bn_finalize_wide_kernel(const float* __restrict__ partial, int rows, int c, int c_pad, double count,
                                                                const float* __restrict__ gamma, const float* __restrict__ beta, float eps,
                                                                float momentum, float* __restrict__ rmean, float* __restrict__ rvar,
                                                                float* __restrict__ ss) {
  constexpr int CB = 8, PARTS = 1024 / CB;
  __shared__ double sh[PARTS][CB][2];
  const int cl = threadIdx.x & (CB - 1), rl = threadIdx.x / CB;
  const int ch = blockIdx.x * CB + cl;
  double s1 = 0, s2 = 0;
  if (ch < c) {
    int r = rl;
    for (; r + 3 * PARTS < rows; r += 4 * PARTS) {
      const float a0 = partial[(size_t)r * 2 * c_pad + ch], b0 = partial[(size_t)r * 2 * c_pad + c_pad + ch];
      const float a1 = partial[(size_t)(r + PARTS) * 2 * c_pad + ch], b1 = partial[(size_t)(r + PARTS) * 2 * c_pad + c_pad + ch];
      const float a2 = partial[(size_t)(r + 2 * PARTS) * 2 * c_pad + ch], b2 = partial[(size_t)(r + 2 * PARTS) * 2 * c_pad + c_pad + ch];
      const float a3 = partial[(size_t)(r + 3 * PARTS) * 2 * c_pad + ch], b3 = partial[(size_t)(r + 3 * PARTS) * 2 * c_pad + c_pad + ch];
      s1 += ((double)a0 + (double)a1) + ((double)a2 + (double)a3);
      s2 += ((double)b0 + (double)b1) + ((double)b2 + (double)b3);
    }
    for (; r < rows; r += PARTS) {
      s1 += (double)partial[(size_t)r * 2 * c_pad + ch];
      s2 += (double)partial[(size_t)r * 2 * c_pad + c_pad + ch];
    }
  }
  sh[rl][cl][0] = s1;
  sh[rl][cl][1] = s2;
  __syncthreads();
  double t1 = 0, t2 = 0;
  if (rl < 8) {
#pragma unroll
    for (int q = 0; q < PARTS / 8; ++q) {
      t1 += sh[rl * (PARTS / 8) + q][cl][0];
      t2 += sh[rl * (PARTS / 8) + q][cl][1];
    }
  }
  __syncthreads();
  if (rl < 8) {
    sh[rl][cl][0] = t1;
    sh[rl][cl][1] = t2;
  }
  __syncthreads();
  if (rl == 0 && ch < c) {
    s1 = 0;
    s2 = 0;
#pragma unroll
    for (int q = 0; q < 8; ++q) {
      s1 += sh[q][cl][0];
      s2 += sh[q][cl][1];
    }
    bn_finalize_channel(s1, s2, count, ch, c, gamma, beta, eps, momentum, rmean, rvar, ss);
  }
}

__global__ __launch_bounds__(256) void bn_partial_kernel(const float* __restrict__ partial, int rows, int c_pad, int chunk, int c_out,
                                                         float* __restrict__ out) {
  const int ch = blockIdx.x * 32 + (threadIdx.x & 31);
  const int r0 = blockIdx.y * chunk;
  float s1, s2;
  bn_fold_rows<float>(partial, r0, min(rows, r0 + chunk), c_pad, ch, ch < c_out, s1, s2);
  if (threadIdx.x < 32 && ch < c_out) {
    out[(size_t)blockIdx.y * 2 * c_out + ch] = s1;
    out[(size_t)blockIdx.y * 2 * c_out + c_out + ch] = s2;
  }
// ... 182 lines not shown
                                                                bf16_t* __restrict__ dz, int dz_ld, float* __restrict__ dgamma,
                                                                float* __restrict__ dbeta, int pix_per_block, int groups, int gshift) {
  const RowLane t = row_lane(c, groups, gshift);
  const int c0 = t.c0, npl = t.npl;
  const float inv = 1.0f / (float)pixels;
  if (blockIdx.x == 0 && blockIdx.y == 0 && dgamma)
    for (int ch = threadIdx.x; ch < c; ch += 256) {
      dbeta[ch] += sums[ch];
      dgamma[ch] += sums[c + ch];
    }
  if (!t.live) return;
  float sc[8], sh[8], mu[8], is[8], m1[8], m2[8];
#pragma unroll
  for (int k = 0; k < 8; ++k) {
    sc[k] = ss[c0 + k];
    sh[k] = ss[c + c0 + k];
    mu[k] = ss[2 * c + c0 + k];
    is[k] = ss[3 * c + c0 + k];
    m1[k] = sums[c0 + k] * inv;
    m2[k] = sums[c + c0 + k] * inv;
  }
  const long long mA = (long long)blockIdx.x * pix_per_block, mB = min(pixels, mA + pix_per_block);
  for (long long m = mA + t.pl; m < mB; m += U * npl) {
    uint4 gu[U], hu[U], zu[U];
#pragma unroll
    for (int u = 0; u < U; ++u) {
      const long long mm = m + (long long)u * npl;
      if (mm < mB) {
        gu[u] = *(const uint4*)(g1 + mm * g1_ld + c0);
        zu[u] = *(const uint4*)(z + mm * z_ld + c0);
        if (g2) hu[u] = *(const uint4*)(g2 + mm * g2_ld + c0);
      }
    }
#pragma unroll
    for (int u = 0; u < U; ++u) {
      const long long mm = m + (long long)u * npl;
      if (mm >= mB) break;
      f32x8 g = unpack8(gu[u]);
      if (g2) add8(g, unpack8(hu[u]));
      const f32x8 zz = unpack8(zu[u]);
      *(uint4*)(dz + mm * dz_ld + c0) = pack8(bn_dz8(bn_dy8(g, zz, sc, sh, slope), zz, sc, mu, is, m1, m2));
    }
  }
}

__global__ __launch_bounds__(256) void upsample2x_fwd_kernel(const bf16_t* __restrict__ x, int x_ld, int n, int h, int w, int c,
                                                             bf16_t* __restrict__ out, int out_ld) {
  const int groups = c >> 3;
  const long long total = (long long)n * (2 * h) * (2 * w) * groups;
  for (long long i = blockIdx.x * 256ll + threadIdx.x; i < total; i += (long long)gridDim.x * 256) {
    const int g = (int)(i % groups);
    const long long p = i / groups;
    const int ox = (int)(p % (2 * w)), oy = (int)((p / (2 * w)) % (2 * h)), b = (int)(p / ((long long)4 * w * h));
    const uint4 v = *(const uint4*)(x + ((long long)(b * h + (oy >> 1)) * w + (ox >> 1)) * x_ld + g * 8);
    *(uint4*)(out + p * out_ld + g * 8) = v;
  }
}

__global__ __launch_bounds__(256) void upsample2x_bwd_kernel(const bf16_t* __restrict__ gq, int g_ld, int n, int h, int w, int c,
                                                             bf16_t* __restrict__ out, int out_ld) {
  const int groups = c >> 3;
  const long long total = (long long)n * h * w * groups;
  for (long long i = blockIdx.x * 256ll + threadIdx.x; i < total; i += (long long)gridDim.x * 256) {
    const int g = (int)(i % groups);
    const long long p = i / groups;
    const int x = (int)(p % w), y = (int)((p / w) % h), b = (int)(p / ((long long)w * h));
    f32x8 a;
#pragma unroll
    for (int k = 0; k < 8; ++k) a.v[k] = 0.f;
#pragma unroll
    for (int dy = 0; dy < 2; ++dy)
#pragma unroll
      for (int dx = 0; dx < 2; ++dx) add8(a, unpack8(*(const uint4*)(gq + ((long long)(b * 2 * h + 2 * y + dy) * (2 * w) + 2 * x + dx) * g_ld + g * 8)));
    *(uint4*)(out + p * out_ld + g * 8) = pack8(a);
  }
}

__global__ __launch_bounds__(256) void add_kernel(const bf16_t* __restrict__ a, int a_ld, const bf16_t* __restrict__ b, int b_ld, int c,
                                                  long long pixels, bf16_t* __restrict__ out, int out_ld) {
  const int groups = c >> 3;
  const long long total = pixels * groups;
  for (long long i = blockIdx.x * 256ll + threadIdx.x; i < total; i += (long long)gridDim.x * 256) {
    const long long m = i / groups;
    const int c0 = (int)(i - m * groups) << 3;
    f32x8 v = unpack8(*(const uint4*)(a + m * a_ld + c0));
    add8(v, unpack8(*(const uint4*)(b + m * b_ld + c0)));
    *(uint4*)(out + m * out_ld + c0) = pack8(v);
  }
}

template <bool OUT_BF16>
__global__ __launch_bounds__(256) void nchw_to_nhwc_kernel(const float* __restrict__ x, int n, int c, int hw, void* __restrict__ out, int out_ld) {
  const long long total = (long long)n * hw;
  for (long long i = blockIdx.x * 256ll + threadIdx.x; i < total; i += (long long)gridDim.x * 256) {
    const long long b = i / hw, p = i - b * hw;
    for (int ch = 0; ch < c; ++ch) {
      const float v = x[(b * c + ch) * hw + p];
      if (OUT_BF16) ((bf16_t*)out)[i * out_ld + ch] = f2s(v);
      else ((float*)out)[i * out_ld + ch] = v;
    }
  }
}

template <bool IN_BF16>
__global__ __launch_bounds__(256) void nhwc_to_nchw_kernel(const void* __restrict__ x, int x_ld, int n, int c, int hw, float* __restrict__ out) {
  const long long total = (long long)n * c * hw;
  for (long long i = blockIdx.x * 256ll + threadIdx.x; i < total; i += (long long)gridDim.x * 256) {
    const long long p = i % hw;
    const int ch = (int)((i / hw) % c);
    const long long b = i / ((long long)hw * c);
    const long long src = (b * hw + p) * x_ld + ch;
    out[i] = IN_BF16 ? s2f(((const bf16_t*)x)[src]) : ((const float*)x)[src];
  }
}

struct RowsGeom {
  int groups, gshift, slabs, ppb, blocks;
};
inline bool rows_geom(int c, long long pixels, RowsGeom* g) {
  if (c <= 0 || c % 8 != 0 || pixels <= 0) return false;
  g->groups = min(c / 8, 256);
  g->slabs = (c / 8 + g->groups - 1) / g->groups;
  int sh = 0;
  while ((1 << sh) < g->groups) ++sh;
  g->gshift = (1 << sh) == g->groups ? sh : -1;
  const int npl = 256 / g->groups;
  long long per = (long long)npl * 16;
  long long nb = (pixels + per - 1) / per;
  if (nb > 16384) {
    per = ((pixels + 16383) / 16384 + npl - 1) / npl * npl;
    nb = (pixels + per - 1) / per;
  }
  if (per > 0x7FFFFFFFll) return false;
  g->ppb = (int)per;
  g->blocks = (int)nb;
  return true;
}

inline int grid_for(long long total) { return (int)min((long long)256 * 16, (total + 255) / 256); }

}


#if !MI355_F16
__global__ __launch_bounds__(256) void sgd_kernel(float* __restrict__ w, float* __restrict__ g, float* __restrict__ mom, long long n4, long long n,
                                                   float lr, float momentum, float dampening, float wd, float gscale, int nesterov, int first,
                                                   int zero_grad, const int* __restrict__ skip) {
  const long long stride = (long long)gridDim.x * blockDim.x;
  if (skip && *skip) {
    if (zero_grad)
      for (long long i = (long long)blockIdx.x * blockDim.x + threadIdx.x; i < n; i += stride) g[i] = 0.f;
    return;
  }
  for (long long i = (long long)blockIdx.x * blockDim.x + threadIdx.x; i < n4; i += stride) {
    float4 wv = ((const float4*)w)[i], gv = ((const float4*)g)[i], mv = ((const float4*)mom)[i];
    float* wp = (float*)&wv; float* gp = (float*)&gv; float* mp = (float*)&mv;
#pragma unroll
    for (int j = 0; j < 4; ++j) {
      float d = gp[j] * gscale + wd * wp[j];
      if (momentum != 0.f) {
        mp[j] = first ? d : momentum * mp[j] + (1.f - dampening) * d;
        d = nesterov ? d + momentum * mp[j] : mp[j];
      }
      wp[j] -= lr * d;
    }
    ((float4*)w)[i] = wv;
    ((float4*)mom)[i] = mv;
    if (zero_grad) ((float4*)g)[i] = make_float4(0.f, 0.f, 0.f, 0.f);
  }
  for (long long i = n4 * 4 + (long long)blockIdx.x * blockDim.x + threadIdx.x; i < n; i += stride) {
    float d = g[i] * gscale + wd * w[i];
    if (momentum != 0.f) {
      mom[i] = first ? d : momentum * mom[i] + (1.f - dampening) * d;
      d = nesterov ? d + momentum * mom[i] : mom[i];
    }
    w[i] -= lr * d;
    if (zero_grad) g[i] = 0.f;
  }
}

__global__ __launch_bounds__(256) void adam_kernel(float* __restrict__ w, float* __restrict__ g, float* __restrict__ m, float* __restrict__ v, long long n,
                                                    float lr, float b1, float b2, float eps, float wd, float gscale, float bc1, float bc2_sqrt,
                                                    int zero_grad, const int* __restrict__ skip) {
  const long long stride = (long long)gridDim.x * blockDim.x;
  if (skip && *skip) {
    if (zero_grad)
      for (long long i = (long long)blockIdx.x * blockDim.x + threadIdx.x; i < n; i += stride) g[i] = 0.f;
    return;
  }
  for (long long i = (long long)blockIdx.x * blockDim.x + threadIdx.x; i < n; i += stride) {
    const float wi = w[i];
    const float d = g[i] * gscale + wd * wi;
    const float mi = b1 * m[i] + (1.f - b1) * d;
    const float vi = b2 * v[i] + (1.f - b2) * d * d;
    m[i] = mi;
    v[i] = vi;
    const float denom = sqrtf(vi) / bc2_sqrt + eps;
    w[i] = wi - (lr / bc1) * (mi / denom);
    if (zero_grad) g[i] = 0.f;
  }
}

__global__ __launch_bounds__(256) void nonfinite_kernel(const float* __restrict__ g, long long n4, long long n, int* __restrict__ flag) {
  const long long stride = (long long)gridDim.x * blockDim.x;
  bool bad = false;
  for (long long i = (long long)blockIdx.x * blockDim.x + threadIdx.x; i < n4; i += stride) {
    const float4 v = ((const float4*)g)[i];
    const float t = (v.x - v.x) + (v.y - v.y) + (v.z - v.z) + (v.w - v.w);
    bad |= !(t == 0.f);
  }
  for (long long i = n4 * 4 + (long long)blockIdx.x * blockDim.x + threadIdx.x; i < n; i += stride) bad |= !((g[i] - g[i]) == 0.f);
  if (__ballot(bad) != 0ull && (threadIdx.x & 63) == 0) *flag = 1;
}

#endif

#if !MI355_F16
static void bn_fold_many_rows(const float*& partial, int32_t& rows, int c_pad, void* stream) {
  if (rows <= 256) return;
  const int chunks = 64, chunk = (rows + chunks - 1) / chunks;
  float* spare = const_cast<float*>(partial) + (size_t)rows * 2 * c_pad;
  hipLaunchKernelGGL(bn_partial_kernel, dim3((c_pad + 31) / 32, chunks), dim3(256), 0, S(stream), partial, rows, c_pad, chunk, c_pad, spare);
  partial = spare;
  rows = chunks;
}
#endif

extern "C" {

#if !MI355_F16
int mi355det_bn_finalize(const float* stats, int32_t rows, int32_t c, int32_t c_pad, int64_t count, const float* gamma, const float* beta, float eps,
                         float momentum, float* running_mean, float* running_var, float* scale_shift, void* stream) {
  if (c <= 0 || rows <= 0 || count <= 0) return fail(MI355DET_EINVAL, "%s: bad arguments", "bn_finalize");
  if (rows > 32 && rows <= 8192) {
    hipLaunchKernelGGL(bn_finalize_wide_kernel, dim3((c + 7) / 8), dim3(1024), 0, S(stream), stats, rows, c, c_pad, (double)count, gamma, beta, eps,
                       momentum, running_mean, running_var, scale_shift);
    return check_launch("bn_finalize");
  }
  bn_fold_many_rows(stats, rows, c_pad, stream);
  hipLaunchKernelGGL(bn_finalize_kernel, dim3((c + 31) / 32), dim3(256), 0, S(stream), stats, rows, c, c_pad, (double)count, gamma, beta, eps,
                     momentum, running_mean, running_var, scale_shift);
  return check_launch("bn_finalize");
}

int mi355det_bn_bwd_sum_partials(const float* partials, int32_t rows, int32_t c, int32_t c_pad, float* sums, void* stream) {
  if (c <= 0 || rows <= 0 || c_pad < c) return fail(MI355DET_EINVAL, "%s: bad arguments", "bn_bwd_sum_partials");
  bn_fold_many_rows(partials, rows, c_pad, stream);
  hipLaunchKernelGGL(bn_partial_kernel, dim3((c + 31) / 32), dim3(256), 0, S(stream), partials, rows, c_pad, rows, c, sums);
  return check_launch("bn_bwd_sum_partials");
}

int mi355det_bn_fold_partials_f64(const float* stats, int32_t rows, int32_t c, int32_t c_pad, double* sums64, void* stream) {
  if (c <= 0 || rows <= 0 || c_pad < c || !stats || !sums64) return fail(MI355DET_EINVAL, "%s: bad arguments", "bn_fold_partials_f64");
  bn_fold_many_rows(stats, rows, c_pad, stream);
  hipLaunchKernelGGL(bn_fold_f64_kernel, dim3((c_pad + 31) / 32), dim3(256), 0, S(stream), stats, rows, c, c_pad, sums64);
  return check_launch("bn_fold_partials_f64");
}

int mi355det_bn_finalize_f64(const double* sums64, int32_t c, int32_t c_pad, int64_t count, const float* gamma, const float* beta, float eps,
                             float momentum, float* running_mean, float* running_var, float* scale_shift, void* stream) {
  if (c <= 0 || c_pad < c || count <= 0 || !sums64) return fail(MI355DET_EINVAL, "%s: bad arguments", "bn_finalize_f64");
  hipLaunchKernelGGL(bn_finalize_f64_kernel, dim3((c + 255) / 256), dim3(256), 0, S(stream), sums64, c, c_pad, (double)count, gamma, beta, eps, momentum,
                     running_mean, running_var, scale_shift);
  return check_launch("bn_finalize_f64");
}

int mi355det_bn_eval_scale_shift(int32_t c, const float* gamma, const float* beta, const float* running_mean, const float* running_var, float eps,
                                 float* scale_shift, void* stream) {
  if (c <= 0) return fail(MI355DET_EINVAL, "%s: bad arguments", "bn_eval");
  hipLaunchKernelGGL(bn_eval_kernel, dim3((c + 255) / 256), dim3(256), 0, S(stream), c, gamma, beta, running_mean, running_var, eps, scale_shift);
  return check_launch("bn_eval");
}

#endif

int mi355det_bn_act_fwd(const void* z, int32_t z_ld, const float* scale_shift, int32_t c, int64_t pixels, float slope, const void* residual,
                        int32_t res_ld, void* out, int32_t out_ld, void* stream) {
  RowsGeom g;
  if (!rows_geom(c, pixels, &g)) return fail(MI355DET_EINVAL, "%s: channels must be a multiple of 8", "bn_act_fwd");
  hipLaunchKernelGGL(bn_act_fwd_rows_kernel<4>, dim3(g.blocks, g.slabs), dim3(256), 0, S(stream), (const bf16_t*)z, z_ld, scale_shift, c,
                     (long long)pixels, slope, (const bf16_t*)residual, res_ld, (bf16_t*)out, out_ld, g.ppb, g.groups, g.gshift);
  return check_launch("bn_act_fwd");
}

struct BnReduceGeom {
  int gb, slabs, blocks;
  long long ppb;
};
static BnReduceGeom bn_reduce_geom(int c, long long pixels) {
  const int groups = c / 8;
  BnReduceGeom g;
  g.gb = groups >= 32 ? 16 : (groups > 8 ? 8 : 1);
  while (g.gb * 2 <= groups && g.gb < 8) g.gb *= 2;
  g.slabs = (groups + g.gb - 1) / g.gb;
  const int npl = 256 / g.gb;
  g.ppb = (long long)npl * 32;
  long long blocks = (pixels + g.ppb - 1) / g.ppb;
  const long long cap = 512 / g.slabs > 64 ? 512 / g.slabs : 64;
  if (blocks > cap) {
    g.ppb = ((pixels + cap - 1) / cap + npl * 4 - 1) / (npl * 4) * (npl * 4);
    blocks = (pixels + g.ppb - 1) / g.ppb;
  }
  g.blocks = (int)blocks;
  return g;
}

size_t mi355det_bn_act_bwd_reduce_workspace(int32_t c, int64_t pixels) {
  if (c <= 0 || c % 8 != 0 || pixels <= 0) return 0;
  const BnReduceGeom g = bn_reduce_geom(c, pixels);
  return (size_t)g.slabs * g.blocks * (size_t)(2 * g.gb * 8) * sizeof(float);
}

static int bn_reduce_launch(const void* g1, int32_t g1_ld, const void* g2, int32_t g2_ld, const void* z, int32_t z_ld, const float* scale_shift, int32_t c,
                            int64_t pixels, float slope, float* sums, void* workspace, size_t workspace_bytes, void* stream, const char* what) {
  if (c <= 0 || c % 8 != 0) return fail(MI355DET_EINVAL, "%s: channels must be a multiple of 8 (got c=%lld)", what, c);
  const BnReduceGeom g = bn_reduce_geom(c, pixels);
  float* part = nullptr;
  if (workspace) {
    if (g.blocks > 512 || workspace_bytes < mi355det_bn_act_bwd_reduce_workspace(c, pixels) || ((uintptr_t)workspace & 15))
      return fail(MI355DET_EINVAL, "%s: workspace too small or misaligned (%lld bytes given)", what, (long long)workspace_bytes);
    part = (float*)workspace;
  }
  hipLaunchKernelGGL(bn_bwd_reduce_kernel, dim3(g.blocks, g.slabs), dim3(256), 0, S(stream), (const bf16_t*)g1, g1_ld, (const bf16_t*)g2, g2_ld,
                     (const bf16_t*)z, z_ld, scale_shift, c, (long long)pixels, slope, sums, (int)g.ppb, g.gb, part);
  if (part) {
    const int cb = g.gb * 8;
    hipLaunchKernelGGL(bn_bwd_fold_rows_kernel, dim3((2 * cb + 31) / 32, g.slabs), dim3(256), 0, S(stream), (const float*)part, g.blocks, cb, c, sums);
  }
  return check_launch(what);
// ... 107 lines not shown
```

### object_detectors_amd/csrc/f16_names.h

```cpp
#pragma once
#define mi355det_conv_autotune_mode mi355det_conv_autotune_mode_f16
#define mi355det_conv_dgrad mi355det_conv_dgrad_f16
#define mi355det_conv_dgrad_bn mi355det_conv_dgrad_bn_f16
#define mi355det_conv_dgrad_bn_rows mi355det_conv_dgrad_bn_rows_f16
#define mi355det_conv_dgrad_mask mi355det_conv_dgrad_mask_f16
#define mi355det_conv_dgrad_workspace mi355det_conv_dgrad_workspace_f16
#define mi355det_conv_dgrad_ws mi355det_conv_dgrad_ws_f16
#define mi355det_conv_fwd mi355det_conv_fwd_f16
#define mi355det_conv_fwd_ex mi355det_conv_fwd_ex_f16
#define mi355det_conv_stats_rows mi355det_conv_stats_rows_f16
#define mi355det_debug_ptr mi355det_debug_ptr_f16
#define mi355det_debug_set mi355det_debug_set_f16
#define mi355det_dgrad_pack_elems mi355det_dgrad_pack_elems_f16
#define mi355det_pack_table_build mi355det_pack_table_build_f16
#define mi355det_pack_table_bytes mi355det_pack_table_bytes_f16
#define mi355det_pack_weights mi355det_pack_weights_f16
#define mi355det_pack_weights_batched mi355det_pack_weights_batched_f16
#define mi355det_stem_im2col mi355det_stem_im2col_f16
#define mi355det_unpack_wgrad mi355det_unpack_wgrad_f16
#define mi355det_conv_wgrad mi355det_conv_wgrad_f16
#define mi355det_conv_wgrad_autotune mi355det_conv_wgrad_autotune_f16
#define mi355det_conv_wgrad_workspace mi355det_conv_wgrad_workspace_f16
#define mi355det_add_bf16 mi355det_add_bf16_f16
#define mi355det_bn_act_bwd_apply mi355det_bn_act_bwd_apply_f16
#define mi355det_bn_act_bwd_reduce mi355det_bn_act_bwd_reduce_f16
#define mi355det_bn_act_bwd_reduce_det mi355det_bn_act_bwd_reduce_det_f16
#define mi355det_bn_act_bwd_reduce_workspace mi355det_bn_act_bwd_reduce_workspace_f16
#define mi355det_bn_act_fwd mi355det_bn_act_fwd_f16
#define mi355det_nchw_f32_to_nhwc mi355det_nchw_f32_to_nhwc_f16
#define mi355det_nhwc_to_nchw_f32 mi355det_nhwc_to_nchw_f32_f16
#define mi355det_upsample2x_bwd mi355det_upsample2x_bwd_f16
#define mi355det_upsample2x_fwd mi355det_upsample2x_fwd_f16
#define mi355det_stem_bwd_apply_wgrad mi355det_stem_bwd_apply_wgrad_f16
#define mi355det_stem_bwd_finish mi355det_stem_bwd_finish_f16
#define mi355det_stem_bwd_fused mi355det_stem_bwd_fused_f16
#define mi355det_stem_bwd_reduce mi355det_stem_bwd_reduce_f16
#define mi355det_stem_fwd_apply mi355det_stem_fwd_apply_f16
#define mi355det_stem_fwd_stats mi355det_stem_fwd_stats_f16
#define mi355det_stem_rows mi355det_stem_rows_f16
#define mi355det_stem_l1_fwd mi355det_stem_l1_fwd_f16
#define mi355det_stem_l1_fwd_eval mi355det_stem_l1_fwd_eval_f16
#define mi355det_stem_l1_rows mi355det_stem_l1_rows_f16
#define mi355det_internal_dgrad_s2 mi355det_internal_dgrad_s2_f16
#define igemm8_launch igemm8_launch_f16
#define igemm8_set_dbg igemm8_set_dbg_f16
#define igemm8_applicable igemm8_applicable_f16
#define igemm8_set_dbg_mode igemm8_set_dbg_mode_f16
#define g_wgrad_general g_wgrad_general_f16
#define g_wgrad_force_dbg g_wgrad_force_dbg_f16
#define g_conv_strict g_conv_strict_f16
#define g_wgrad8_off g_wgrad8_off_f16
#define g_wgrad_ablate g_wgrad_ablate_f16
#define g_dgrad_s2_off g_dgrad_s2_off_f16
#define pack_batched_kernel pack_batched_kernel_f16
#define splitk_reduce_kernel splitk_reduce_kernel_f16
```

### object_detectors_amd/optim.py

```python
import torch

from ._lib import check, lib


def _stream():
    return torch.cuda.current_stream().cuda_stream


class _Flat(torch.optim.Optimizer):
    def __init__(self, flat_w, flat_g, defaults):
        if flat_w.dtype != torch.float32 or flat_g.dtype != torch.float32 or flat_w.numel() != flat_g.numel():
            raise ValueError("flat parameter and gradient buffers must be fp32 and equally sized")
        if not flat_w.is_cuda:
            raise ValueError("mi355det optimizers run on the GPU buffers of an engine (no CPU path)")
        self.flat_w, self.flat_g = flat_w, flat_g
        super().__init__([flat_w], defaults)
        self.steps = 0

    @classmethod
    def for_engine(cls, engine, **kw):
        return cls(engine.flat_w, engine.flat_g, **kw)

    def zero_grad(self, set_to_none=False):
        self.flat_g.zero_()


class FlatSGD(_Flat):

    def __init__(self, flat_w, flat_g, lr=1e-3, momentum=0.0, dampening=0.0, weight_decay=0.0, nesterov=False):
        super().__init__(flat_w, flat_g, dict(lr=lr, momentum=momentum, dampening=dampening, weight_decay=weight_decay, nesterov=nesterov))
        self.momentum_buf = torch.zeros_like(flat_w)

    @torch.no_grad()
    def step(self, closure=None, grad_scale=1.0, zero_grad=False, skip_flag=None):
        g = self.param_groups[0]
        st = lib().mi355det_sgd_step_guarded(self.flat_w.data_ptr(), self.flat_g.data_ptr(), self.momentum_buf.data_ptr(), self.flat_w.numel(),
                                             float(g["lr"]), float(g["momentum"]), float(g["dampening"]), float(g["weight_decay"]),
                                             float(grad_scale), int(bool(g["nesterov"])), int(self.steps == 0), int(zero_grad),
                                             None if skip_flag is None else skip_flag.data_ptr(), _stream())
        check(st, "sgd_step")
        self.steps += 1


    def reference_state_dict(self, engine):
        g = self.param_groups[0]
        tensors = engine.reference_parameter_tensors(self.momentum_buf)
        state = {i: {"momentum_buffer": t} for i, t in enumerate(tensors)} if self.steps > 0 and g["momentum"] != 0 else {}
        group = {k: g[k] for k in ("lr", "momentum", "dampening", "weight_decay", "nesterov")}
        group["params"] = list(range(len(tensors)))
        return {"state": state, "param_groups": [group]}

    def load_reference_state_dict(self, engine, sd):
        g = sd["param_groups"][0]
        for k in ("lr", "momentum", "dampening", "weight_decay", "nesterov"):
            if k in g:
                self.param_groups[0][k] = g[k]
        if sd["state"]:
            n = len(g["params"])
            bufs = [sd["state"][i]["momentum_buffer"] for i in range(n)]
            engine.load_reference_parameter_tensors(bufs, self.momentum_buf)
            self.steps = max(self.steps, 1)
        else:
            self.momentum_buf.zero_()
            self.steps = 0


class FlatAdam(_Flat):

    def __init__(self, flat_w, flat_g, lr=1e-3, betas=(0.9, 0.999), eps=1e-8, weight_decay=0.0):
        super().__init__(flat_w, flat_g, dict(lr=lr, betas=betas, eps=eps, weight_decay=weight_decay))
        self.exp_avg = torch.zeros_like(flat_w)
        self.exp_avg_sq = torch.zeros_like(flat_w)

    @torch.no_grad()
    def step(self, closure=None, grad_scale=1.0, zero_grad=False, skip_flag=None):
        g = self.param_groups[0]
        self.steps += 1
        st = lib().mi355det_adam_step_guarded(self.flat_w.data_ptr(), self.flat_g.data_ptr(), self.exp_avg.data_ptr(), self.exp_avg_sq.data_ptr(),
                                              self.flat_w.numel(), float(g["lr"]), float(g["betas"][0]), float(g["betas"][1]), float(g["eps"]),
                                              float(g["weight_decay"]), float(grad_scale), self.steps, int(zero_grad),
                                              None if skip_flag is None else skip_flag.data_ptr(), _stream())
        check(st, "adam_step")

    def reference_state_dict(self, engine):
        g = self.param_groups[0]
        m, v = engine.reference_parameter_tensors(self.exp_avg), engine.reference_parameter_tensors(self.exp_avg_sq)
        state = {i: {"step": torch.tensor(float(self.steps)), "exp_avg": a, "exp_avg_sq": b} for i, (a, b) in enumerate(zip(m, v))} if self.steps else {}
        group = {"lr": g["lr"], "betas": tuple(g["betas"]), "eps": g["eps"], "weight_decay": g["weight_decay"], "amsgrad": False,
                 "params": list(range(len(m)))}
        return {"state": state, "param_groups": [group]}

    def load_reference_state_dict(self, engine, sd):
        g = sd["param_groups"][0]
        for k in ("lr", "betas", "eps", "weight_decay"):
            if k in g:
                self.param_groups[0][k] = g[k]
        if sd["state"]:
            n = len(g["params"])
            engine.load_reference_parameter_tensors([sd["state"][i]["exp_avg"] for i in range(n)], self.exp_avg)
            engine.load_reference_parameter_tensors([sd["state"][i]["exp_avg_sq"] for i in range(n)], self.exp_avg_sq)
            self.steps = int(sd["state"][0]["step"])
        else:
            self.exp_avg.zero_()
            self.exp_avg_sq.zero_()
            self.steps = 0


class DynamicLossScaler:

    def __init__(self, init_scale=2.0 ** 16, scale_factor=2.0, scale_window=2000, min_loss_scale=None, max_loss_scale=2.0 ** 24, enabled=True):
        self.loss_scale = float(init_scale) if enabled else 1.0
        self.scale_factor, self.scale_window = float(scale_factor), int(scale_window)
        self.min_loss_scale, self.max_loss_scale = min_loss_scale, max_loss_scale
        self.enabled = enabled
        self.unskipped = 0
        self.skipped_steps = 0
        self._flag = None

    def step(self, optimizer, zero_grad=False):
        if not self.enabled:
            optimizer.step(zero_grad=zero_grad)
            return True
        g = optimizer.flat_g
        if self._flag is None or self._flag.device != g.device:
            self._flag = torch.zeros(1, dtype=torch.int32, device=g.device)
        self._flag.zero_()
        check(lib().mi355det_grad_nonfinite(g.data_ptr(), g.numel(), self._flag.data_ptr(), _stream()), "grad_nonfinite")
        optimizer.step(grad_scale=1.0 / self.loss_scale, zero_grad=zero_grad, skip_flag=self._flag)
        overflow = bool(self._flag.item())
        if overflow:
            optimizer.steps -= 1
            self.skipped_steps += 1
            self.loss_scale = self.loss_scale / self.scale_factor
            if self.min_loss_scale is not None:
                self.loss_scale = max(self.loss_scale, self.min_loss_scale)
            self.unskipped = 0
        else:
            self.unskipped += 1
            if self.unskipped == self.scale_window:
                self.loss_scale = min(self.max_loss_scale, self.loss_scale * self.scale_factor)
                self.unskipped = 0
        return not overflow

    def state_dict(self):
        return {"loss_scale": self.loss_scale, "unskipped": self.unskipped}

    def load_state_dict(self, sd):
        self.loss_scale, self.unskipped = float(sd["loss_scale"]), int(sd["unskipped"])
```

### object_detectors_amd/plan_core.py

```python
import contextlib
import ctypes as C

import torch

from . import _lib, tune
from ._lib import check


def _vp(t, byte_off=0):
    return C.c_void_p(t.data_ptr() + byte_off) if t is not None else None


def comm_hook(*a):
    raise RuntimeError("marker only")


class Act:

    def __init__(self, buf, n, h, w, c, ld, ch_off=0, needs_grad=True):
        self.buf, self.n, self.h, self.w, self.c, self.ld, self.ch_off = buf, n, h, w, c, ld, ch_off
        self.needs_grad = needs_grad
        self.grad = None
        self.grad_written = False
        self.parts = []
        self.conv_consumers = 0

    @property
    def ptr(self):
        return C.c_void_p(self.buf.data_ptr() + 2 * self.ch_off)

    @property
    def pixels(self):
        return self.n * self.h * self.w

    def slice(self, c0, c):
        return Act(self.buf, self.n, self.h, self.w, c, self.ld, self.ch_off + c0)


def check_images(images, why=""):
    if images.dim() != 4 or images.shape[1] != 3 or not images.is_cuda:
        raise ValueError("expected a CUDA tensor [n,3,H,W]")
    n, _, H, W = images.shape
    if H % 32 or W % 32:
        raise ValueError("input size must be a multiple of 32" + why)
    return n, H, W


def cached_plan(eng, key, build, training, dp):
    p = eng.plans.pop(key, None)
    if p is None:
        while len(eng.plans) >= eng.MAX_PLANS:
            torch.cuda.current_stream().synchronize()
            eng.plans.pop(next(iter(eng.plans)))
        p = tune.plan_build(build, share=None if dp else False)
        if training:
            for gs in getattr(eng, "grad_syncs", ()):
                gs.install(p)
    eng.plans[key] = p
    return p


def build_pack_table(L, eng, specs, shape_of, need_dgrad):
    items = (_lib.PackItem * max(1, len(specs)))()
    for i, s in enumerate(specs):
        wf, wd = eng.packed[s.name]
        items[i].w = eng.params[s.name + ".weight"].data_ptr()
        items[i].w_fwd = wf.data_ptr()
        items[i].w_dgrad = wd.data_ptr() if (need_dgrad and wd is not None) else None
        items[i].shape, items[i].cout_pad = shape_of(s)
        items[i].w_is_ohwi = 1
    ne, nb = C.c_int32(0), C.c_int32(0)
    nbytes = L.mi355det_pack_table_bytes(items, len(specs), C.byref(ne), C.byref(nb))
    host = torch.empty(max(nbytes, 1), dtype=torch.uint8)
    check(L.mi355det_pack_table_build(items, len(specs), C.c_void_p(host.data_ptr()), nbytes), "pack_table_build")
    return host.to(eng.device), ne.value, nb.value


class PlanBase:

    def __init__(self, eng, L, n, H, W, training, stream):
        self.eng, self.L, self.n, self.H, self.W, self.training = eng, L, n, H, W, training
        self.stream = C.c_void_p(stream)
        self.fwd, self.bwd, self.pack = [], [], []
        self.keep = []
        self.ops = []
        self.layers = {}
        self.grad_bufs = []

    def _run(self, calls):
        for fn, args in calls:
            if fn is comm_hook:
                args[0](*args[1:])
                continue
            st = fn(*args)
            if st != 0:
                check(st, fn.__name__)

    def build_pack_table(self, specs, shape_of, need_dgrad):
        self.pack_table, ne, nb = build_pack_table(self.L, self.eng, specs, shape_of, need_dgrad)
        self.pack.append((self.L.mi355det_pack_weights_batched, (_vp(self.pack_table), ne, nb, self.stream)))

    @contextlib.contextmanager
    def autotuning(self):
        self.L.mi355det_conv_autotune_mode(1)
        try:
            yield
        finally:
            self.L.mi355det_conv_autotune_mode(0)

    def autotune_wgrads(self, convs):
        ws_ptr, ws_bytes = _vp(self.wgrad_ws), self.wgrad_ws.numel()
        for shp, x_ptr, dy_ptr, dw in convs:
            st = self.L.mi355det_conv_wgrad_autotune(C.byref(shp), x_ptr, dy_ptr, _vp(dw), ws_ptr, ws_bytes, self.stream)
            if st < 0:
                check(st, "conv_wgrad_autotune")
        torch.cuda.synchronize()
        self.eng.flat_g.zero_()


class BackwardSchedule:

    def __init__(self, plan, dev, dtype, dz_elems, ws_bytes, streams=None, new_event=None):
        self.L, self.bwd = plan.L, plan.bwd
        self.main, self.side = streams or (torch.cuda.current_stream(dev), torch.cuda.Stream(device=dev))
        self.new_event = new_event or torch.cuda.Event
        self.side_ptr = C.c_void_p(self.side.cuda_stream)
        plan.side = self.side
        plan.dz2 = self.dz2 = [torch.zeros(dz_elems, device=dev, dtype=dtype) for _ in range(2)]
        plan.wgrad_ws = torch.empty(max(ws_bytes, 16), device=dev, dtype=torch.uint8)
        self.ws = (_vp(plan.wgrad_ws), plan.wgrad_ws.numel())
        self.wg_done = [None, None]
        self.flip = 0

    def py(self, fn, *a):
        self.bwd.append((comm_hook, (fn,) + a))

    def next_dz(self):
        di, self.flip = self.flip, self.flip ^ 1
        if self.wg_done[di] is not None:
            self.py(self.main.wait_event, self.wg_done[di])
        return di

    def publish(self):
        ev = self.new_event()
        self.py(ev.record, self.main)
        self.py(self.side.wait_event, ev)

    def wgrad(self, shp, x_ptr, dy_ptr, dw, dbias, dz_index=None, record=True, groups=1):
        self.publish()
        if groups > 1:
            assert dbias is None
            self.bwd.append((self.L.mi355det_gconv_wgrad, (C.byref(shp), groups, x_ptr, dy_ptr, _vp(dw)) + self.ws + (self.side_ptr,)))
        else:
            self.bwd.append((self.L.mi355det_conv_wgrad, (C.byref(shp), x_ptr, dy_ptr, _vp(dw), _vp(dbias)) + self.ws + (self.side_ptr,)))
        if record:
            ev = self.new_event()
            self.py(ev.record, self.side)
            if dz_index is not None:
                self.wg_done[dz_index] = ev

    def close(self, plan):
        ev = self.new_event()
        self.py(ev.record, self.side)
        self.py(self.main.wait_event, ev)
        plan.side_stream = self.side


class GradAccumulator:

    def __init__(self, L, dev, dtype, plan, dgrad_call):
        self.L, self.dev, self.dtype, self.dgrad_call = L, dev, dtype, dgrad_call
        self.bwd, self.grad_bufs, self.stream = plan.bwd, plan.grad_bufs, plan.stream

    def dense(self, a):
        g = Act(torch.zeros((a.n, a.h, a.w, a.c), device=self.dev, dtype=self.dtype), a.n, a.h, a.w, a.c, a.c)
        self.grad_bufs.append(g.buf)
        return g

    def grad_of(self, a):
        if a.grad is None:
            a.grad = self.dense(a)
        return a.grad

    def _add(self, a, p, q, out):
        self.bwd.append((self.L.mi355det_add_bf16, (p.ptr, p.ld, q.ptr, q.ld, a.c, a.pixels, out.ptr, out.ld, self.stream)))

    def _drain(self, a):
        while a.parts:
            self._add(a, a.grad, a.parts.pop(0), a.grad)

    def add_tensor(self, x, t):
        if not x.needs_grad:
            return
        if x.grad_written:
            self._add(x, x.grad, t, x.grad)
        else:
            x.parts.append(t)

    def add_dgrad(self, x, shp, dy_ptr, wd, call=None):
        if not x.needs_grad:
            return
        g, call = self.grad_of(x), call or self.dgrad_call
        if x.grad_written:
            self.bwd.append(call(shp, dy_ptr, wd, g, g.ptr, g.ld))
            return
        r = x.parts.pop(0) if x.parts else None
        self.bwd.append(call(shp, dy_ptr, wd, g, r.ptr if r else None, r.ld if r else 0))
        x.grad_written = True
        self._drain(x)

    def finalize(self, a):
        if a.grad_written:
            return a.grad
        if not a.parts:
            return None
        if len(a.parts) == 1:
            a.grad = a.parts.pop(0)
        else:
            a.grad = self.dense(a)
            self._add(a, a.parts.pop(0), a.parts.pop(0), a.grad)
            self._drain(a)
        a.grad_written = True
        return a.grad
```

### object_detectors_amd/yolo/nets/engine.py

```python
import ctypes as C
import math
import os

import torch

from ... import _lib, ops
from ..._lib import lib
from ...plan_core import Act, BackwardSchedule, GradAccumulator, PlanBase, _vp, cached_plan, check_images, comm_hook

BLOCKS = {"darknet_21": [1, 1, 2, 2, 1], "darknet_53": [1, 2, 8, 8, 4]}
SLOPE = 0.1
BN_EPS, BN_MOM = 1e-5, 0.1


class ConvSpec:
    def __init__(self, name, cin, cout, k, stride, bn=True, bias=False):
        self.name, self.cin, self.cout, self.k, self.stride, self.bn, self.bias = name, cin, cout, k, stride, bn, bias


def arch(backbone="darknet_53", na=3, nc=80):
    specs = [ConvSpec("backbone.conv1", 3, 32, 3, 1)]
    inpl = 32
    for li, (planes, nb) in enumerate(zip([(32, 64), (64, 128), (128, 256), (256, 512), (512, 1024)], BLOCKS[backbone]), 1):
        p = f"backbone.layer{li}"
        specs.append(ConvSpec(p + ".ds_conv", inpl, planes[1], 3, 2))
        inpl = planes[1]
        for b in range(nb):
            specs.append(ConvSpec(f"{p}.residual_{b}.conv1", inpl, planes[0], 1, 1))
            specs.append(ConvSpec(f"{p}.residual_{b}.conv2", planes[0], inpl, 3, 1))
    fo = na * (5 + nc)

    def emb(name, fl, cin):
        ch = [(cin, fl[0], 1), (fl[0], fl[1], 3), (fl[1], fl[0], 1), (fl[0], fl[1], 3), (fl[1], fl[0], 1), (fl[0], fl[1], 3)]
        for i, (ci, co, k) in enumerate(ch):
            specs.append(ConvSpec(f"{name}.{i}.conv", ci, co, k, 1))
        specs.append(ConvSpec(name + ".conv_out", fl[1], fo, 1, 1, bn=False, bias=True))
    emb("embedding0", (512, 1024), 1024)
    specs.append(ConvSpec("embedding1_cbl.conv", 512, 256, 1, 1))
    emb("embedding1", (256, 512), 768)
    specs.append(ConvSpec("embedding2_cbl.conv", 256, 128, 1, 1))
    emb("embedding2", (128, 256), 384)
    return specs


def bn_name(conv_name):
    if conv_name == "backbone.conv1":
        return "backbone.bn1"
    if conv_name.endswith(".ds_conv"):
        return conv_name[:-len("ds_conv")] + "ds_bn"
    if conv_name.endswith(".conv1"):
        return conv_name[:-len("conv1")] + "bn1"
    if conv_name.endswith(".conv2"):
        return conv_name[:-len("conv2")] + "bn2"
    return conv_name[:-len("conv")] + "bn"


class YoloV3Engine:
    def __init__(self, backbone="darknet_53", num_anchors=3, num_classes=80, device=None, seed=0, sync_bn=False, process_group=None, storage="bf16",
                 deterministic=True, fuse_bn_reduce=False):
        lib()
        storage = os.environ.get("MI355DET_STORAGE", storage) if storage == "bf16" else storage
        if storage not in ("bf16", "fp16"):
            raise ValueError("storage must be 'bf16' or 'fp16'")
        self.storage = storage
        self.deterministic = bool(deterministic)
        self.fuse_bn_reduce = bool(fuse_bn_reduce)
        self.L = _lib.storage_lib(storage)
        self.adt = torch.float16 if storage == "fp16" else torch.bfloat16
        self.grad_fmt = 2 if storage == "fp16" else 1
        self.sync_bn, self.process_group = bool(sync_bn), process_group
        if self.sync_bn and process_group is None:
            import torch.distributed as dist
            if dist.is_available() and dist.is_initialized() and dist.get_world_size() > 1:
                self.process_group = dist.new_group()
        self.device = device or torch.device("cuda", torch.cuda.current_device())
        self.backbone, self.na, self.nc = backbone, num_anchors, num_classes
        self.head_c = num_anchors * (5 + num_classes)
        self.head_ld = ops.pad_to(self.head_c, 32)
        self._static_epoch = 1
        self._frozen = False
        self.specs = arch(backbone, num_anchors, num_classes)
        self.by_name = {s.name: s for s in self.specs}
        self._layout_params()
        self.reset_parameters(seed)
        self.plans = {}
        self.training = True
        self.num_batches_tracked = 0

    def freeze_inference(self, on=True):
        self._static_epoch += 1
        self._frozen = bool(on)

    def _weights_changed(self):
        self._static_epoch += 1

    def _layout_params(self):
        off = 0
        self.pviews = {}
        order = []
        for s in self.specs:
            if s.name == "backbone.conv1":
                shape = (32, 32)
            elif not s.bn:
                shape = (ops.pad_to(s.cout, 32), s.k, s.k, s.cin)
            else:
                shape = (s.cout, s.k, s.k, s.cin)
            n = math.prod(shape)
            order.append((s.name + ".weight", off, n, shape))
            off += ops.pad_to(n, 64)
            if s.bias:
                order.append((s.name + ".bias", off, s.cout, (s.cout,)))
                off += ops.pad_to(s.cout, 64)
            if s.bn:
                b = bn_name(s.name)
                for suffix in (".weight", ".bias"):
                    order.append((b + suffix, off, s.cout, (s.cout,)))
                    off += ops.pad_to(s.cout, 64)
        self.flat_w = torch.zeros(off, device=self.device, dtype=torch.float32)
        self.flat_g = torch.zeros(off, device=self.device, dtype=torch.float32)
        self.param_order = order
        self.params, self.grads = {}, {}
        for name, o, n, shape in order:
            self.params[name] = self.flat_w[o:o + n].view(shape)
            self.grads[name] = self.flat_g[o:o + n].view(shape)
        self.buffers = {}
        for s in self.specs:
            if s.bn:
                b = bn_name(s.name)
                self.buffers[b + ".running_mean"] = torch.zeros(s.cout, device=self.device)
                self.buffers[b + ".running_var"] = torch.ones(s.cout, device=self.device)
        self.packed = {}
        for s in self.specs:
            shp = self._wshape(s, 1, 8, 8)
            cp = ops.cout_pad_of(shp.cout)
            wf = torch.zeros(cp * shp.ksize * shp.ksize * shp.cin, device=self.device, dtype=self.adt)
            wd = None
            if s.name != "backbone.conv1":
                wd = torch.zeros(self.L.mi355det_dgrad_pack_elems(C.byref(shp)), device=self.device, dtype=self.adt)
            self.packed[s.name] = (wf, wd)

    def _wshape(self, s, n, h, w, in_ld=None, out_ld=None):
        if s.name == "backbone.conv1":
            return ops.conv_shape(n, h, w, 32, 32, 1, 1, in_ld, out_ld)
        cout = s.cout if s.bn else ops.pad_to(s.cout, 32)
        return ops.conv_shape(n, h, w, s.cin, cout, s.k, s.stride, in_ld, out_ld)

    def reset_parameters(self, seed=0):
        g = torch.Generator(device="cpu").manual_seed(seed)
        for s in self.specs:
            w = self.params[s.name + ".weight"]
            if s.name.startswith("backbone."):
                std = math.sqrt(2.0 / (s.k * s.k * s.cout))
                t = torch.randn((s.cout, s.cin, s.k, s.k), generator=g) * std
            else:
                bound = 1.0 / math.sqrt(s.cin * s.k * s.k)
                t = (torch.rand((s.cout, s.cin, s.k, s.k), generator=g) * 2 - 1) * bound
            self._set_weight_oihw(s, t)
            if s.bias:
                bound = 1.0 / math.sqrt(s.cin * s.k * s.k)
                self.params[s.name + ".bias"].copy_((torch.rand(s.cout, generator=g) * 2 - 1) * bound)
            if s.bn:
                b = bn_name(s.name)
                self.params[b + ".weight"].fill_(1.0)
                self.params[b + ".bias"].zero_()
            del w
        self._weights_changed()

    def flat_views(self, flat):
        if flat.numel() != self.flat_w.numel():
            raise ValueError("buffer does not have the engine's flat layout")
        return {name: flat[o:o + n].view(shape) for name, o, n, shape in self.param_order}

    def _set_weight_oihw(self, s, t, dst=None):
        w = (dst or self.params)[s.name + ".weight"]
        t = t.to(self.device, torch.float32)
        if s.name == "backbone.conv1":
            w.zero_()
            w[:, :27] = t.permute(0, 2, 3, 1).reshape(32, 27)
        elif not s.bn:
            w.zero_()
            w[:s.cout] = t.permute(0, 2, 3, 1)
        else:
            w.copy_(t.permute(0, 2, 3, 1))

    def _get_weight_oihw(self, s, src=None):
        w = (src or self.params)[s.name + ".weight"]
        if s.name == "backbone.conv1":
            return w[:, :27].reshape(32, 3, 3, 3).permute(0, 3, 1, 2).contiguous()
        if not s.bn:
            return w[:s.cout].permute(0, 3, 1, 2).contiguous()
        return w.permute(0, 3, 1, 2).contiguous()

    def load_reference_state_dict(self, sd):
        for s in self.specs:
            self._set_weight_oihw(s, sd[s.name + ".weight"])
            if s.bias:
                self.params[s.name + ".bias"].copy_(sd[s.name + ".bias"])
            if s.bn:
                b = bn_name(s.name)
                self.params[b + ".weight"].copy_(sd[b + ".weight"])
                self.params[b + ".bias"].copy_(sd[b + ".bias"])
                for k in (".running_mean", ".running_var"):
                    if b + k in sd:
                        self.buffers[b + k].copy_(sd[b + k])
                if b + ".num_batches_tracked" in sd:
                    self.num_batches_tracked = int(sd[b + ".num_batches_tracked"])
        self._weights_changed()

    def reference_parameter_tensors(self, flat):
        sd = self.reference_state_dict(src=self.flat_views(flat), params_only=True)
        return list(sd.values())

    def load_reference_parameter_tensors(self, tensors, flat):
        dst = self.flat_views(flat)
        names = list(self.reference_state_dict(params_only=True).keys())
        if len(names) != len(tensors):
            raise ValueError(f"expected {len(names)} parameter tensors, got {len(tensors)}")
        byname = dict(zip(names, tensors))
        for s in self.specs:
            self._set_weight_oihw(s, byname[s.name + ".weight"], dst)
            if s.bias:
                dst[s.name + ".bias"].copy_(byname[s.name + ".bias"])
            if s.bn:
                b = bn_name(s.name)
                dst[b + ".weight"].copy_(byname[b + ".weight"])
                dst[b + ".bias"].copy_(byname[b + ".bias"])
        self._weights_changed()

    def reference_state_dict(self, grads=False, src=None, params_only=False):
        out = {}
        if src is None:
            src = self.grads if grads else self.params
        else:
            grads = True
        for s in self.specs:
            out[s.name + ".weight"] = self._get_weight_oihw(s, src)
            if s.bias:
                out[s.name + ".bias"] = src[s.name + ".bias"].clone()
            if s.bn:
                b = bn_name(s.name)
                out[b + ".weight"] = src[b + ".weight"].clone()
                out[b + ".bias"] = src[b + ".bias"].clone()
                if not grads and not params_only:
                    for k in (".running_mean", ".running_var"):
                        out[b + k] = self.buffers[b + k].clone()
                    out[b + ".num_batches_tracked"] = torch.tensor(self.num_batches_tracked, dtype=torch.int64)
        return out
# ... 225 lines not shown
            self.fwd.append(img_call(L.mi355det_stem_fwd_apply, (_vp(wf), _vp(ss), SLOPE, a.ptr, a.ld, n, H, W, self.stream)))
        rec = dict(kind="stem", name=name, spec=s, x=None, a=a, res=None, z=None, ss=ss, pixels=pixels, rows=rows, img_call=img_call, fused_l1=fused)
        a.producer = rec
        self.ops.append(rec)
        self.layers[name] = rec
        return a

    def _build_backward(self):
        eng, L, dev = self.eng, self.eng.L, self.eng.device
        bf = eng.adt
        self.fuse_bn_reduce = eng.fuse_bn_reduce
        ws_need = max(L.mi355det_conv_wgrad_workspace(C.byref(r["shp_f"] if r["kind"] == "out" else r["shp"]))
                      for r in self.ops if r["kind"] in ("cbl", "out"))
        sched = BackwardSchedule(self, dev, bf, self.dz_elems, ws_need)
        self.dz = self.dz2[0]
        py = sched.py
        nsum = sum(2 * r["shp"].cout for r in self.ops if r["kind"] == "cbl") + 64
        self.sums_all = torch.zeros(nsum, device=dev, dtype=torch.float32)
        sum_off = [0]
        red_need = max([L.mi355det_bn_act_bwd_reduce_workspace(r["shp"].cout, r["pixels"]) for r in self.ops if r["kind"] == "cbl"] + [1024])
        self.bn_red_ws = torch.zeros(red_need, device=dev, dtype=torch.uint8)
        red_ptr, red_bytes = _vp(self.bn_red_ws), self.bn_red_ws.numel()

        acc = GradAccumulator(L, dev, bf, self, lambda shp, dy_ptr, wd, g, rptr, rld: (
            L.mi355det_conv_dgrad, (C.byref(shp), dy_ptr, _vp(wd), g.ptr, rptr, rld, self.stream)))

        def emit_dgrad(shp, dy_ptr, wd, x):
            g = acc.grad_of(x)
            if g.ld != shp.in_ld:
                shp = _lib.ConvShape(shp.n, shp.h, shp.w, shp.cin, shp.ho, shp.wo, shp.cout, shp.ksize, shp.stride, shp.pad, g.ld,
                                     shp.out_ld)
                self.keep.append(shp)
            prod, call = getattr(x, "producer", None), None
            if (not x.grad_written and prod is not None and prod.get("z") is not None and x.conv_consumers == 1 and len(x.parts) <= 1
                    and self.fuse_bn_reduce):
                rows = L.mi355det_conv_dgrad_bn_rows(C.byref(shp))
                cpad = ops.pad_to(x.c, 32)
                part = torch.zeros((rows + 64, 2, cpad), device=dev, dtype=torch.float32)
                prod["bn_partials"] = (part, rows, cpad)

                def call(shp, dy_ptr, wd, g, rptr, rld):
                    return (L.mi355det_conv_dgrad_bn, (C.byref(shp), dy_ptr, _vp(wd), g.ptr, rptr, rld, _vp(prod["z"]), x.c, _vp(prod["ss"]), SLOPE,
                                                       _vp(part), self.stream))
            acc.add_dgrad(x, shp, dy_ptr, wd, call)

        self.bwd_marks = []
        first_off = {name: o for name, o, _n, _s in eng.param_order}
        for rec in reversed(self.ops):
            if rec["kind"] in ("out", "cbl", "stem"):
                self._mark_name = rec["name"]
            if rec["kind"] == "stem":
                name, a, ss, rows, img_call = rec["name"], rec["a"], rec["ss"], rec["rows"], rec["img_call"]
                assert a.grad is not None and a.grad_written and not a.parts, name
                g, b = a.grad, bn_name(name)
                wf, _ = eng.packed[name]
                sums = self.sums_all[sum_off[0]:sum_off[0] + 64]
                sum_off[0] += 64
                slab = torch.zeros((rows, 2048), device=dev, dtype=torch.float32)
                ag = torch.zeros(2048, device=dev, dtype=torch.float32)
                self.keep += [slab, ag]
                self.bwd.append(img_call(L.mi355det_stem_bwd_fused, (_vp(wf), _vp(ss), SLOPE, g.ptr, g.ld, _vp(slab), _vp(ag), _vp(sums),
                                                                     self.n, self.H, self.W, self.stream)))
                if self.sync_world > 1:
                    py(self._sync_avg, sums)
                self.bwd.append((L.mi355det_stem_bwd_finish, (_vp(wf), _vp(ss), _vp(ag), _vp(sums), self.n * self.H * self.W,
                                                              _vp(eng.grads[name + ".weight"]), _vp(eng.grads[b + ".weight"]),
                                                              _vp(eng.grads[b + ".bias"]), self.stream)))
                sched.publish()
            elif rec["kind"] == "out":
                shp, shp_f, x, k, name = rec["shp"], rec["shp_f"], rec["x"], rec["k"], rec["name"]
                _, wd = eng.packed[name]
                dy = _vp(self.head_grads[k])
                sched.wgrad(shp_f, x.ptr, dy, eng.grads[name + ".weight"], eng.grads[name + ".bias"], record=False)
                emit_dgrad(shp, dy, wd, x)
            elif rec["kind"] == "up":
                x, cat, c_up, skip_to = rec["x"], rec["cat"], rec["c_up"], rec["skip_to"]
                assert cat.grad is not None and cat.grad_written
                gup = cat.grad.slice(0, c_up)
                gx = acc.grad_of(x)
                self.bwd.append((L.mi355det_upsample2x_bwd, (gup.ptr, gup.ld, x.n, x.h, x.w, x.c, gx.ptr, gx.ld, self.stream)))
                x.grad_written = True
                acc.add_tensor(skip_to, cat.grad.slice(c_up, cat.c - c_up))
            else:
                name, shp, x, a, res, z, ss, pixels = (rec[k] for k in ("name", "shp", "x", "a", "res", "z", "ss", "pixels"))
                assert a.grad is not None and a.grad_written and not a.parts, name
                g = a.grad
                b = bn_name(name)
                sums = self.sums_all[sum_off[0]:sum_off[0] + 2 * shp.cout]
                sum_off[0] += 2 * shp.cout
                if res is not None:
                    acc.add_tensor(res, g)
                if "bn_partials" in rec:
                    part, prows, cpad = rec["bn_partials"]
                    self.bwd.append((L.mi355det_bn_bwd_sum_partials, (_vp(part), prows, shp.cout, cpad, _vp(sums), self.stream)))
                elif eng.deterministic:
                    self.bwd.append((L.mi355det_bn_act_bwd_reduce_det, (g.ptr, g.ld, None, 0, _vp(z), shp.cout, _vp(ss), shp.cout, pixels, SLOPE,
                                                                        _vp(sums), red_ptr, red_bytes, self.stream)))
                else:
                    self.bwd.append((L.mi355det_bn_act_bwd_reduce, (g.ptr, g.ld, None, 0, _vp(z), shp.cout, _vp(ss), shp.cout, pixels, SLOPE,
                                                                    _vp(sums), self.stream)))
                if self.sync_world > 1:
                    py(self._sync_avg, sums)
                di = rec["dz_index"] = sched.next_dz()
                dzb = self.dz2[di]
                self.bwd.append((L.mi355det_bn_act_bwd_apply, (g.ptr, g.ld, None, 0, _vp(z), shp.cout, _vp(ss), _vp(sums), None, shp.cout,
                                                               pixels, SLOPE, _vp(dzb), shp.cout, _vp(eng.grads[b + ".weight"]),
                                                               _vp(eng.grads[b + ".bias"]), self.stream)))
                sched.wgrad(shp, x.ptr, _vp(dzb), eng.grads[name + ".weight"], None, dz_index=di)
                _, wd = eng.packed[name]
                emit_dgrad(shp, _vp(dzb), wd, x)
            if rec["kind"] in ("out", "cbl", "stem"):
                self.bwd_marks.append((len(self.bwd), first_off[rec["name"] + ".weight"]))
        sched.close(self)

    def _autotune(self):
        eng = self.eng
        saved = {k: v.clone() for k, v in eng.buffers.items()}
        img = torch.randn((self.n, 3, self.H, self.W), device=eng.device)
        self._set_image(img)
        for g in self.head_grads:
            g.normal_(0, 1e-2)
        with self.autotuning():
            self._run(self.pack)
            self._run(self.fwd)
            self._run(self.bwd)

        def wgrad_of(r):
            shp, dy = (r["shp"], self.dz) if r["kind"] == "cbl" else (r["shp_f"], self.head_grads[r["k"]])
            return shp, r["x"].ptr, _vp(dy), eng.grads[r["name"] + ".weight"]
        self.autotune_wgrads(wgrad_of(r) for r in self.ops if r["kind"] in ("cbl", "out"))
        for k, v in saved.items():
            eng.buffers[k].copy_(v)
        self.zero_head_grads()

    def _autotune_eval(self):
        img = torch.randn((self.n, 3, self.H, self.W), device=self.eng.device)
        self._set_image(img)
        self._run(self.pack)
        self._run(self.fwd_const)
        with self.autotuning():
            self._run(self.fwd)
        torch.cuda.synchronize()

    def _set_image(self, images):
        self._img = images
        ptr = C.c_void_p(images.data_ptr())
        for a in self.img_args:
            a[0] = ptr

    def run_forward(self, images):
        self._set_image(images)
        eng = self.eng
        if self.training:
            eng._weights_changed()
            self._run(self.pack)
        elif not (eng._frozen and self._const_epoch == eng._static_epoch):
            self._run(self.pack)
            self._run(self.fwd_const)
            self._const_epoch = eng._static_epoch if eng._frozen else -1
        self._run(self.fwd)
        if self.training:
            eng.num_batches_tracked += 1

    def head_outputs(self):
        c = self.eng.head_c
        return [h[..., :c].permute(0, 3, 1, 2) for h in self.heads]

    def head_grad_views(self):
        c = self.eng.head_c
        return [g[..., :c].permute(0, 3, 1, 2) for g in self.head_grads]

    def zero_head_grads(self):
        for g in self.head_grads:
            g.zero_()

    def load_head_grads(self, grads):
        c = self.eng.head_c
        for dst, g in zip(self.head_grads, grads):
            dst[..., :c].copy_(g.permute(0, 2, 3, 1))

    def run_backward(self):
        self.eng.flat_g.zero_()
        self.sums_all.zero_()
        self.side.wait_stream(torch.cuda.current_stream())
        self._run(self.bwd)
```

Before: 1158 images/s.

## Fuse SGD update with bf16 weight repacking into a single kernel

Adds a fused kernel that applies the SGD momentum update to the fp32 master weights and writes the packed bf16 forward and dgrad weight layouts in the same pass. The next training forward then skips its separate pack launch when the packs are already current. This removes one full read of the master weights and a kernel launch per step, at the cost of a more complex pack table covering the whole flat buffer, including regions that are not conv weights. It is enabled by default through an environment variable, with a fallback to the old path for Adam or when no plan exists.

Result: no change. 1163 images/s (median of 6 runs) (+0.5%).

```diff
diff --git a/include/mi355det.h b/include/mi355det.h
--- a/include/mi355det.h
+++ b/include/mi355det.h
@@ -270,6 +270,13 @@
 size_t mi355det_pack_table_bytes(const mi355det_pack_item* items, int32_t n, int32_t* n_entries, int32_t* n_blocks);
 int mi355det_pack_table_build(const mi355det_pack_item* items, int32_t n, void* host_table, size_t host_bytes);
 int mi355det_pack_weights_batched(const void* dev_table, int32_t n_entries, int32_t n_blocks, void* stream);
+size_t mi355det_sgd_pack_table_bytes(const mi355det_pack_item* items, int32_t n, const float* flat_w, int64_t flat_n,
+                                     int32_t* n_entries, int32_t* n_blocks);
+int mi355det_sgd_pack_table_build(const mi355det_pack_item* items, int32_t n, const float* flat_w, int64_t flat_n,
+                                  void* host_table, size_t host_bytes);
+int mi355det_sgd_pack_step(const void* dev_table, int32_t n_entries, int32_t n_blocks, float* w, float* g, float* momentum_buf,
+                           float lr, float momentum, float dampening, float weight_decay, float grad_scale, int nesterov,
+                           int first_step, int zero_grad, const int* skip_flag, void* stream);
 int mi355det_unpack_wgrad(const mi355det_conv_shape* s, const float* dw, float* grad, void* stream);
 
 size_t mi355det_gconv_pack_elems(const mi355det_conv_shape* s, int32_t groups);
diff --git a/include/mi355det_f16.h b/include/mi355det_f16.h
--- a/include/mi355det_f16.h
+++ b/include/mi355det_f16.h
@@ -22,6 +22,9 @@
 size_t mi355det_pack_table_bytes_f16(const mi355det_pack_item* items, int32_t n, int32_t* n_entries, int32_t* n_blocks);
 int mi355det_pack_weights_f16(const mi355det_conv_shape* s, const float* w, int w_is_ohwi, void* w_fwd, int32_t cout_pad, void* w_dgrad, void* stream);
 int mi355det_pack_weights_batched_f16(const void* dev_table, int32_t n_entries, int32_t n_blocks, void* stream);
+int mi355det_sgd_pack_step_f16(const void* dev_table, int32_t n_entries, int32_t n_blocks, float* w, float* g, float* momentum_buf, float lr, float momentum, float dampening, float weight_decay, float grad_scale, int nesterov, int first_step, int zero_grad, const int* skip_flag, void* stream);
+int mi355det_sgd_pack_table_build_f16(const mi355det_pack_item* items, int32_t n, const float* flat_w, int64_t flat_n, void* host_table, size_t host_bytes);
+size_t mi355det_sgd_pack_table_bytes_f16(const mi355det_pack_item* items, int32_t n, const float* flat_w, int64_t flat_n, int32_t* n_entries, int32_t* n_blocks);
 int mi355det_stem_im2col_f16(const float* img, void* out, int32_t n, int32_t h, int32_t w, void* stream);
 int mi355det_unpack_wgrad_f16(const mi355det_conv_shape* s, const float* dw, float* grad, void* stream);
 int mi355det_conv_wgrad_f16(const mi355det_conv_shape* s, const void* x, const void* dy, float* dw, float* dbias, void* workspace, size_t workspace_bytes, void* stream);
diff --git a/object_detectors_amd/_lib.py b/object_detectors_amd/_lib.py
--- a/object_detectors_amd/_lib.py
+++ b/object_detectors_amd/_lib.py
@@ -137,6 +137,9 @@
     "mi355det_pack_table_bytes": (sz, [P(PackItem), i32, P(i32), P(i32)]),
     "mi355det_pack_table_build": (C.c_int, [P(PackItem), i32, vp, sz]),
     "mi355det_pack_weights_batched": (C.c_int, [vp, i32, i32, vp]),
+    "mi355det_sgd_pack_table_bytes": (sz, [P(PackItem), i32, vp, i64, P(i32), P(i32)]),
+    "mi355det_sgd_pack_table_build": (C.c_int, [P(PackItem), i32, vp, i64, vp, sz]),
+    "mi355det_sgd_pack_step": (C.c_int, [vp, i32, i32, vp, vp, vp] + [C.c_float] * 5 + [C.c_int] * 3 + [vp, vp]),
     "mi355det_unpack_wgrad": (C.c_int, [P(ConvShape), vp, vp, vp]),
     "mi355det_gconv_pack_elems": (sz, [P(ConvShape), i32]),
     "mi355det_gconv_pack_weights": (C.c_int, [P(ConvShape), i32, vp, C.c_int, vp, vp, vp]),
diff --git a/object_detectors_amd/csrc/conv_kernels.hip b/object_detectors_amd/csrc/conv_kernels.hip
--- a/object_detectors_amd/csrc/conv_kernels.hip
+++ b/object_detectors_amd/csrc/conv_kernels.hip
@@ -1,8 +1,13 @@
 #include "common.h"
-
+#include "sgd_update.h"
+
+#include <algorithm>
+#include <cstdint>
 #include <cstdlib>
 
 #include <unordered_map>
+#include <utility>
+#include <vector>
 
 #include "tune_record.h"
 #include "tune_timing.h"
@@ -1230,43 +1235,58 @@
   return check_launch("pack_weights");
 }
 
+enum { PACK_TILE = 0, PACK_FILL = 1, PACK_PLAIN = 2 };
 struct PackEntry {
   const float* src;
-  bf16_t* dst;
+  bf16_t* fwd;
+  bf16_t* dg;
   long long s_co, s_ci, s_t;
-  int total, rows_valid, cin, kk, ntaps, mode, cdim, cob;
-  int taps[9];
-  int ncib, ncob, pad1;
+  long long start, total;
+  long long d_base[9], c_base[9];
+  int d_rs[9], c_rs[9];
+  int mode, rows, cin, kk, cob, ncib, ncob;
+  int vec;
+  int run, stride;
 };
 #define PACK_CHUNK 4096
 
-__global__ __launch_bounds__(256) void pack_batched_kernel(const PackEntry* __restrict__ entries, const int2* __restrict__ blocks) {
+extern "C++" {
+namespace {
+
+template <bool STEP>
+__device__ __forceinline__ void pack_piece(const PackEntry* __restrict__ entries, const int2* __restrict__ blocks, float* __restrict__ w,
+                                           float* __restrict__ g, float* __restrict__ mom, const SgdArgs& a, bool skip) {
   const int2 bt = blocks[blockIdx.x];
-  const PackEntry e = entries[bt.x];
-  if (e.mode == 2) {
-    const long long n0 = (long long)2 * e.cin * 2 * e.cdim;
-    const int end = min(e.total, bt.y + PACK_CHUNK);
-    for (int i = bt.y + threadIdx.x; i < end; i += 256) {
-      const int py = i >= n0;
-      const long long j = py ? i - n0 : i;
-      const int T = py ? 4 : 2;
-      const int co = (int)(j % e.cdim), tap = (int)((j / e.cdim) % T), r = (int)(j / ((long long)e.cdim * T));
-      const int px = r / e.cin, ci = r - px * e.cin;
-      const int oy = py ? tap >> 1 : 0, ox = py ? tap & 1 : tap;
-      const int kh = s2cat_k(py, oy), kw = s2cat_k(px, ox);
-      float v = 0.f;
-      if (kh >= 0 && kw >= 0) v = e.src[co * e.s_co + ci * e.s_ci + (kh * 3 + kw) * e.s_t];
-      e.dst[i] = f2s(v);
-    }
+  const PackEntry& e = entries[bt.x];
+  const int tid = threadIdx.x;
+  if (e.mode == PACK_FILL) {
+    if (skip) return;
+    const long long lo = (long long)bt.y * PACK_CHUNK, hi = min(e.total, lo + PACK_CHUNK);
+    for (long long i = lo + tid; i < hi; i += 256) e.fwd[(i / e.run) * e.stride + i % e.run] = 0;
     return;
   }
-  if (e.mode == 0) {
-    const int end = min(e.total, bt.y + PACK_CHUNK);
-    for (int i = bt.y + threadIdx.x; i < end; i += 256) {
-      const int c = i % e.cin, t = (i / e.cin) % e.kk, co = i / (e.cin * e.kk);
-      float v = 0.f;
-      if (co < e.rows_valid) v = e.src[co * e.s_co + c * e.s_ci + t * e.s_t];
-      e.dst[i] = f2s(v);
+  if (e.mode == PACK_PLAIN) {
+    if constexpr (STEP) {
+      const long long lo = e.start + (long long)bt.y * PACK_CHUNK, hi = min(e.start + e.total, lo + PACK_CHUNK);
+      const long long va = min(hi, (lo + 3) & ~3ll), vb = va + ((hi - va) & ~3ll);
+      for (long long i = va / 4 + tid; i < vb / 4; i += 256) {
+        if (skip) {
+          if (a.zero_grad) ((float4*)g)[i] = make_float4(0.f, 0.f, 0.f, 0.f);
+          continue;
+        }
+        float4 wv = ((const float4*)w)[i], gv = ((const float4*)g)[i], mv = ((const float4*)mom)[i];
+        float* wp = (float*)&wv; float* gp = (float*)&gv; float* mp = (float*)&mv;
+#pragma unroll
+        for (int j = 0; j < 4; ++j) sgd_update(wp[j], gp[j], mp[j], a);
+        ((float4*)w)[i] = wv;
+        ((float4*)mom)[i] = mv;
+        if (a.zero_grad) ((float4*)g)[i] = make_float4(0.f, 0.f, 0.f, 0.f);
+      }
+      for (long long i = lo + tid; i < hi; i += 256) {
+        if (i >= va && i < vb) continue;
+        if (!skip) sgd_update(w[i], g[i], mom[i], a);
+        if (a.zero_grad) g[i] = 0.f;
+      }
     }
     return;
   }
@@ -1274,111 +1294,204 @@
   int t = bt.y;
   const int co_blk = t % e.ncob;
   t /= e.ncob;
-  const int ci_blk = t % e.ncib, j = t / e.ncib;
-  int tap = e.taps[0];
-#pragma unroll
-  for (int q = 1; q < 9; ++q)
-    if (j == q) tap = e.taps[q];
-  const int cl = threadIdx.x & 31;
-  for (int r = threadIdx.x >> 5; r < e.cob; r += 8) {
-    const int co = co_blk * e.cob + r, ci = ci_blk * 32 + cl;
-    tl[r][cl] = ci < e.rows_valid ? e.src[co * e.s_co + ci * e.s_ci + tap * e.s_t] : 0.f;
-  }
+  const int ci_blk = t % e.ncib, tap = t / e.ncib;
+  const int cob = e.cob, rows = e.rows, cin = e.cin, kk = e.kk;
+  bf16_t* const fwd = e.fwd;
+  if (e.vec) {
+    const long long off = STEP ? e.src - w : 0;
+    const int q = tid & 7, ci = ci_blk * 32 + q * 4;
+    for (int r = tid >> 3; r < cob; r += 32) {
+      const int co = co_blk * cob + r;
+      float4 v = make_float4(0.f, 0.f, 0.f, 0.f);
+      if (co < rows && ci < cin) {
+        const long long i = ((long long)co * kk + tap) * cin + ci;
+        if constexpr (STEP) {
+          float4* const wq = (float4*)(w + off + i); float4* const gq = (float4*)(g + off + i); float4* const mq = (float4*)(mom + off + i);
+          if (skip) {
+            if (a.zero_grad) *gq = v;
+            continue;
+          }
+          v = *wq;
+          float4 gv = *gq, mv = *mq;
+          float* wp = (float*)&v; float* gp = (float*)&gv; float* mp = (float*)&mv;
+#pragma unroll
+          for (int j = 0; j < 4; ++j) sgd_update(wp[j], gp[j], mp[j], a);
+          *wq = v;
+          *mq = mv;
+          if (a.zero_grad) *gq = make_float4(0.f, 0.f, 0.f, 0.f);
+        } else {
+          v = *(const float4*)(e.src + i);
+        }
+        if (fwd) {
+          uint2 u;
+          u.x = f2s(v.x) | ((unsigned)f2s(v.y) << 16);
+          u.y = f2s(v.z) | ((unsigned)f2s(v.w) << 16);
+          *(uint2*)(fwd + i) = u;
+        }
+      }
+      tl[r][q * 4 + 0] = v.x; tl[r][q * 4 + 1] = v.y; tl[r][q * 4 + 2] = v.z; tl[r][q * 4 + 3] = v.w;
+    }
+  } else {
+    const int cl = tid & 31, ci = ci_blk * 32 + cl;
+    for (int r = tid >> 5; r < cob; r += 8) {
+      const int co = co_blk * cob + r;
+      float v = 0.f;
+      if (co < rows && ci < cin) {
+        v = e.src[co * e.s_co + ci * e.s_ci + tap * e.s_t];
+        if (fwd) fwd[((long long)co * kk + tap) * cin + ci] = f2s(v);
+      }
+      tl[r][cl] = v;
+    }
+  }
+  if (!e.dg || skip) return;
   __syncthreads();
-  const int col = threadIdx.x % e.cob;
-  for (int r = threadIdx.x / e.cob; r < 32; r += 256 / e.cob) {
+  const long long d = e.d_base[tap], c = e.c_base[tap];
+  const int d_rs = e.d_rs[tap], c_rs = e.c_rs[tap];
+  const int col = tid % cob, co = co_blk * cob + col;
+  for (int r = tid / cob; r < 32; r += 256 / cob) {
     const long long ci = ci_blk * 32 + r;
-    e.dst[(ci * e.ntaps + j) * e.cdim + co_blk * e.cob + col] = f2s(tl[col][r]);
-  }
-}
-
-size_t mi355det_pack_table_bytes(const mi355det_pack_item* items, int32_t n, int32_t* n_entries, int32_t* n_blocks) {
-  int ne = 0;
-  long long nb = 0;
+    const bf16_t s = f2s(tl[col][r]);
+    if (d >= 0) e.dg[d + ci * d_rs + co] = s;
+    if (c >= 0 && ci < cin) e.dg[c + ci * c_rs + co] = s;
+  }
+}
+
+}
+}
+
+__global__ __launch_bounds__(256) void pack_batched_kernel(const PackEntry* __restrict__ entries, const int2* __restrict__ blocks) {
+  pack_piece<false>(entries, blocks, nullptr, nullptr, nullptr, SgdArgs{}, false);
+}
+
+__global__ __launch_bounds__(256) void sgd_pack_kernel(const PackEntry* __restrict__ entries, const int2* __restrict__ blocks, float* __restrict__ w,
+                                                        float* __restrict__ g, float* __restrict__ mom, const SgdArgs a,
+                                                        const int* __restrict__ skip) {
+  pack_piece<true>(entries, blocks, w, g, mom, a, skip && *skip);
+}
+
+static int pack_table_fill(const mi355det_pack_item* items, int n, const float* flat, long long flat_n, PackEntry* E, int2* B, int* n_entries,
+                           int* n_blocks, const char* who) {
+  int ei = 0;
+  long long bi = 0;
+  auto add = [&](const PackEntry& e, long long blocks) {
+    if (E) {
+      E[ei] = e;
+      for (long long k = 0; k < blocks; ++k) B[bi + k] = make_int2(ei, (int)k);
+    }
+    ++ei;
+    bi += blocks;
+  };
+  auto fill = [&](bf16_t* dst, long long first, long long run, long long stride, long long nruns) {
+    if (run <= 0 || nruns <= 0) return;
+    PackEntry e{};
+    e.mode = PACK_FILL; e.fwd = dst + first; e.run = (int)run; e.stride = (int)stride; e.total = run * nruns;
+    add(e, (e.total + PACK_CHUNK - 1) / PACK_CHUNK);
+  };
+  std::vector<std::pair<long long, long long>> covered;
   for (int i = 0; i < n; ++i) {
     const mi355det_conv_shape* s = &items[i].shape;
-    const int kk = s->ksize * s->ksize;
-    if (items[i].w_fwd) {
-      ++ne;
-      nb += ((long long)items[i].cout_pad * kk * s->cin + PACK_CHUNK - 1) / PACK_CHUNK;
-    }
-    if (items[i].w_dgrad) {
-      const int cin_pad = (s->cin + 31) / 32 * 32;
-      const int classes = s->stride == 1 ? 1 : 4;
-      for (int c = 0; c < classes; ++c) {
-        int ft[9], dy[9], dx[9];
+    if (int e = check_shape(s, who)) return e;
+    if (items[i].w_dgrad && s->cout % 32 != 0) return fail(MI355DET_EINVAL, "%s: dgrad pack needs cout %% 32 == 0", who);
+    if (!items[i].w_fwd && !items[i].w_dgrad) continue;
+    const int kk = s->ksize * s->ksize, cin = s->cin, cout = s->cout;
+    const long long elems = (long long)cout * kk * cin;
+    bf16_t* const wf = (bf16_t*)items[i].w_fwd;
+    bf16_t* const wd = (bf16_t*)items[i].w_dgrad;
+    PackEntry e{};
+    e.mode = PACK_TILE; e.src = items[i].w; e.fwd = wf; e.dg = wd;
+    e.s_co = (long long)cin * kk; e.s_ci = items[i].w_is_ohwi ? 1 : kk; e.s_t = items[i].w_is_ohwi ? cin : 1;
+    e.rows = cout; e.cin = cin; e.kk = kk;
+    e.cob = wd && cout % 64 != 0 ? 32 : 64;
+    e.ncib = (cin + 31) / 32;
+    e.ncob = (cout + e.cob - 1) / e.cob;
+    e.vec = items[i].w_is_ohwi && cin % 4 == 0 && (uintptr_t)items[i].w % 16 == 0 && (uintptr_t)wf % 8 == 0;
+    for (int q = 0; q < 9; ++q) e.d_base[q] = e.c_base[q] = -1;
+    if (flat) {
+      const long long first = items[i].w - flat;
+      if (first < 0 || first + elems > flat_n) return fail(MI355DET_EINVAL, "%s: a master lies outside the flat buffer", who);
+      if (!e.vec) return fail(MI355DET_EINVAL, "%s: needs OHWI masters, cin %% 4 == 0, 16-byte aligned masters and packs", who);
+      covered.push_back({first, first + elems});
+    }
+    if (wd) {
+      const int cin_pad = e.ncib * 32;
+      long long class_off = 0;
+      for (int c = 0; c < (s->stride == 1 ? 1 : 4); ++c) {
+        int ft[9] = {0}, dy[9], dx[9];
         const int nt = dgrad_taps(s, c >> 1, c & 1, ft, dy, dx);
-        ++ne;
-        const int cob = s->cout % 64 == 0 ? 64 : 32;
-        nb += (long long)nt * (cin_pad / 32) * (s->cout / cob);
+        for (int j = 0; j < nt; ++j) {
+          e.d_base[ft[j]] = class_off + (long long)j * cout;
+          e.d_rs[ft[j]] = nt * cout;
+        }
+        class_off += (long long)cin_pad * nt * cout;
       }
       mi355det_conv_shape d = *s;
       d.in_ld = d.cin;
       if (s2cat_eligible(&d)) {
-        ++ne;
-        nb += ((long long)s2cat_elems(&d) + PACK_CHUNK - 1) / PACK_CHUNK;
-      }
-    }
-  }
+        const long long cat = (long long)dgrad_class_elems(s), n0 = (long long)4 * cin * cout;
+        for (int py = 0; py < 2; ++py)
+          for (int px = 0; px < 2; ++px)
+            for (int tp = 0; tp < (py ? 4 : 2); ++tp) {
+              const int T = py ? 4 : 2, kh = s2cat_k(py, py ? tp >> 1 : 0), kw = s2cat_k(px, py ? tp & 1 : tp);
+              const long long at = cat + (py ? n0 : 0) + ((long long)px * cin * T + tp) * cout;
+              if (kh >= 0 && kw >= 0) {
+                e.c_base[kh * 3 + kw] = at;
+                e.c_rs[kh * 3 + kw] = T * cout;
+              }
+            }
+      }
+    }
+    add(e, (long long)kk * e.ncib * e.ncob);
+    if (wf) fill(wf, elems, ((long long)items[i].cout_pad - cout) * kk * cin, 0, 1);
+    if (wd && e.c_base[4] >= 0) {
+      const long long cat = (long long)dgrad_class_elems(s), n0 = (long long)4 * cin * cout;
+      fill(wd, cat + cout, cout, 2 * cout, cin);
+      fill(wd, cat + n0 + cout, cout, 2 * cout, 2 * cin);
+    }
+  }
+  if (flat) {
+    std::sort(covered.begin(), covered.end());
+    long long at = 0;
+    covered.push_back({flat_n, flat_n});
+    for (const auto& r : covered) {
+      if (r.first < at) return fail(MI355DET_EINVAL, "%s: masters overlap", who);
+      if (r.first > at) {
+        PackEntry e{};
+        e.mode = PACK_PLAIN; e.start = at; e.total = r.first - at;
+        add(e, (e.total + PACK_CHUNK - 1) / PACK_CHUNK);
+      }
+      at = r.second;
+    }
+  }
+  if (bi > 0x7FFFFFFFll) return fail(MI355DET_EINVAL, "%s: too many blocks", who);
+  *n_entries = ei;
+  *n_blocks = (int)bi;
+  return 0;
+}
+
+static size_t pack_table_size(const mi355det_pack_item* items, int32_t n, const float* flat, long long flat_n, int32_t* n_entries, int32_t* n_blocks,
+                              const char* who) {
+  int ne = 0, nb = 0;
+  if (pack_table_fill(items, n, flat, flat_n, nullptr, nullptr, &ne, &nb, who)) ne = nb = 0;
   if (n_entries) *n_entries = ne;
-  if (n_blocks) *n_blocks = (int)nb;
+  if (n_blocks) *n_blocks = nb;
   return (size_t)ne * sizeof(PackEntry) + (size_t)nb * sizeof(int2);
 }
 
+static int pack_table_write(const mi355det_pack_item* items, int32_t n, const float* flat, long long flat_n, void* host_table, size_t host_bytes,
+                            const char* who) {
+  int ne = 0, nb = 0;
+  if (int e = pack_table_fill(items, n, flat, flat_n, nullptr, nullptr, &ne, &nb, who)) return e;
+  if (!host_table || host_bytes < (size_t)ne * sizeof(PackEntry) + (size_t)nb * sizeof(int2))
+    return fail(MI355DET_EWORKSPACE, "%s: host table too small", who);
+  return pack_table_fill(items, n, flat, flat_n, (PackEntry*)host_table, (int2*)((char*)host_table + (size_t)ne * sizeof(PackEntry)), &ne, &nb, who);
+}
+
+size_t mi355det_pack_table_bytes(const mi355det_pack_item* items, int32_t n, int32_t* n_entries, int32_t* n_blocks) {
+  return pack_table_size(items, n, nullptr, 0, n_entries, n_blocks, "pack_table_bytes");
+}
+
 int mi355det_pack_table_build(const mi355det_pack_item* items, int32_t n, void* host_table, size_t host_bytes) {
-  int ne = 0, nb = 0;
-  const size_t need = mi355det_pack_table_bytes(items, n, &ne, &nb);
-  if (host_bytes < need) return fail(MI355DET_EWORKSPACE, "%s: host table too small", "pack_table_build");
-  PackEntry* E = (PackEntry*)host_table;
-  int2* B = (int2*)((char*)host_table + (size_t)ne * sizeof(PackEntry));
-  int ei = 0, bi = 0;
-  auto add_blocks = [&](int entry, long long total) {
-    for (long long o = 0; o < total; o += PACK_CHUNK) B[bi++] = make_int2(entry, (int)o);
-  };
-  for (int i = 0; i < n; ++i) {
-    const mi355det_conv_shape* s = &items[i].shape;
-    if (int e = check_shape(s, "pack_table_build")) return e;
-    if (items[i].w_dgrad && s->cout % 32 != 0) return fail(MI355DET_EINVAL, "%s: dgrad pack needs cout %% 32 == 0", "pack_table_build");
-    const int kk = s->ksize * s->ksize;
-    const long long s_co = (long long)s->cin * kk, s_ci = items[i].w_is_ohwi ? 1 : kk, s_t = items[i].w_is_ohwi ? s->cin : 1;
-    if (items[i].w_fwd) {
-      PackEntry& e = E[ei];
-      e = PackEntry{};
-      e.src = items[i].w; e.dst = (bf16_t*)items[i].w_fwd; e.s_co = s_co; e.s_ci = s_ci; e.s_t = s_t;
-      e.total = items[i].cout_pad * kk * s->cin; e.rows_valid = s->cout; e.cin = s->cin; e.kk = kk; e.mode = 0;
-      add_blocks(ei++, e.total);
-    }
-    if (items[i].w_dgrad) {
-      const int cin_pad = (s->cin + 31) / 32 * 32;
-      bf16_t* out = (bf16_t*)items[i].w_dgrad;
-      const int classes = s->stride == 1 ? 1 : 4;
-      for (int c = 0; c < classes; ++c) {
-        int ft[9] = {0}, dy[9], dx[9];
-        const int nt = dgrad_taps(s, c >> 1, c & 1, ft, dy, dx);
-        PackEntry& e = E[ei];
-        e = PackEntry{};
-        e.src = items[i].w; e.dst = out; e.s_co = s_co; e.s_ci = s_ci; e.s_t = s_t;
-        e.total = cin_pad * nt * s->cout; e.rows_valid = s->cin; e.cin = s->cin; e.kk = kk; e.ntaps = nt; e.mode = 1; e.cdim = s->cout;
-        for (int q = 0; q < 9; ++q) e.taps[q] = ft[q];
-        e.cob = s->cout % 64 == 0 ? 64 : 32;
-        e.ncib = cin_pad / 32;
-        e.ncob = s->cout / e.cob;
-        for (int tix = 0; tix < nt * e.ncib * e.ncob; ++tix) B[bi++] = make_int2(ei, tix);
-        ++ei;
-        out += e.total;
-      }
-      mi355det_conv_shape d = *s;
-      d.in_ld = d.cin;
-      if (s2cat_eligible(&d)) {
-        PackEntry& e = E[ei];
-        e = PackEntry{};
-        e.src = items[i].w; e.dst = (bf16_t*)items[i].w_dgrad + dgrad_class_elems(s); e.s_co = s_co; e.s_ci = s_ci; e.s_t = s_t;
-        e.total = (int)s2cat_elems(&d); e.cin = s->cin; e.cdim = s->cout; e.mode = 2;
-        add_blocks(ei++, e.total);
-      }
-    }
-  }
-  return 0;
+  return pack_table_write(items, n, nullptr, 0, host_table, host_bytes, "pack_table_build");
 }
 
 int mi355det_pack_weights_batched(const void* dev_table, int32_t n_entries, int32_t n_blocks, void* stream) {
@@ -1387,6 +1500,31 @@
   const int2* B = (const int2*)((const char*)dev_table + (size_t)n_entries * sizeof(PackEntry));
   hipLaunchKernelGGL(pack_batched_kernel, dim3(n_blocks), dim3(256), 0, S(stream), E, B);
   return check_launch("pack_weights_batched");
+}
+
+size_t mi355det_sgd_pack_table_bytes(const mi355det_pack_item* items, int32_t n, const float* flat_w, int64_t flat_n, int32_t* n_entries,
+                                     int32_t* n_blocks) {
+  if (!flat_w || flat_n <= 0) n = 0, flat_n = 0;
+  return pack_table_size(items, n, flat_w, flat_n, n_entries, n_blocks, "sgd_pack_table_bytes");
+}
+
+int mi355det_sgd_pack_table_build(const mi355det_pack_item* items, int32_t n, const float* flat_w, int64_t flat_n, void* host_table,
+                                  size_t host_bytes) {
+  if (!flat_w || flat_n <= 0) return fail(MI355DET_EINVAL, "%s: no flat buffer", "sgd_pack_table_build");
+  return pack_table_write(items, n, flat_w, flat_n, host_table, host_bytes, "sgd_pack_table_build");
+}
+
+int mi355det_sgd_pack_step(const void* dev_table, int32_t n_entries, int32_t n_blocks, float* w, float* g, float* momentum_buf, float lr,
+                           float momentum, float dampening, float weight_decay, float grad_scale, int nesterov, int first_step, int zero_grad,
+                           const int* skip_flag, void* stream) {
+  if (!dev_table || n_entries <= 0 || n_blocks <= 0) return fail(MI355DET_EINVAL, "%s: bad table", "sgd_pack_step");
+  if (!w || !g || !momentum_buf || ((uintptr_t)w | (uintptr_t)g | (uintptr_t)momentum_buf) % 16 != 0)
+    return fail(MI355DET_EINVAL, "%s: w, g and the momentum buffer must be 16-byte aligned device buffers", "sgd_pack_step");
+  const PackEntry* E = (const PackEntry*)dev_table;
+  const int2* B = (const int2*)((const char*)dev_table + (size_t)n_entries * sizeof(PackEntry));
+  const SgdArgs a{lr, momentum, dampening, weight_decay, grad_scale, nesterov, first_step, zero_grad};
+  hipLaunchKernelGGL(sgd_pack_kernel, dim3(n_blocks), dim3(256), 0, S(stream), E, B, w, g, momentum_buf, a, skip_flag);
+  return check_launch("sgd_pack_step");
 }
 
 int mi355det_unpack_wgrad(const mi355det_conv_shape* s, const float* dw, float* grad, void* stream) {
diff --git a/object_detectors_amd/csrc/elem_kernels.hip b/object_detectors_amd/csrc/elem_kernels.hip
--- a/object_detectors_amd/csrc/elem_kernels.hip
+++ b/object_detectors_amd/csrc/elem_kernels.hip
@@ -1,4 +1,5 @@
 #include "common.h"
+#include "sgd_update.h"
 
 #include <cstdlib>
 
@@ -487,29 +488,18 @@
       for (long long i = (long long)blockIdx.x * blockDim.x + threadIdx.x; i < n; i += stride) g[i] = 0.f;
     return;
   }
+  const SgdArgs a{lr, momentum, dampening, wd, gscale, nesterov, first, zero_grad};
   for (long long i = (long long)blockIdx.x * blockDim.x + threadIdx.x; i < n4; i += stride) {
     float4 wv = ((const float4*)w)[i], gv = ((const float4*)g)[i], mv = ((const float4*)mom)[i];
     float* wp = (float*)&wv; float* gp = (float*)&gv; float* mp = (float*)&mv;
 #pragma unroll
-    for (int j = 0; j < 4; ++j) {
-      float d = gp[j] * gscale + wd * wp[j];
-      if (momentum != 0.f) {
-        mp[j] = first ? d : momentum * mp[j] + (1.f - dampening) * d;
-        d = nesterov ? d + momentum * mp[j] : mp[j];
-      }
-      wp[j] -= lr * d;
-    }
+    for (int j = 0; j < 4; ++j) sgd_update(wp[j], gp[j], mp[j], a);
     ((float4*)w)[i] = wv;
     ((float4*)mom)[i] = mv;
     if (zero_grad) ((float4*)g)[i] = make_float4(0.f, 0.f, 0.f, 0.f);
   }
   for (long long i = n4 * 4 + (long long)blockIdx.x * blockDim.x + threadIdx.x; i < n; i += stride) {
-    float d = g[i] * gscale + wd * w[i];
-    if (momentum != 0.f) {
-      mom[i] = first ? d : momentum * mom[i] + (1.f - dampening) * d;
-      d = nesterov ? d + momentum * mom[i] : mom[i];
-    }
-    w[i] -= lr * d;
+    sgd_update(w[i], g[i], mom[i], a);
     if (zero_grad) g[i] = 0.f;
   }
 }
diff --git a/object_detectors_amd/csrc/f16_names.h b/object_detectors_amd/csrc/f16_names.h
--- a/object_detectors_amd/csrc/f16_names.h
+++ b/object_detectors_amd/csrc/f16_names.h
@@ -16,6 +16,9 @@
 #define mi355det_pack_table_bytes mi355det_pack_table_bytes_f16
 #define mi355det_pack_weights mi355det_pack_weights_f16
 #define mi355det_pack_weights_batched mi355det_pack_weights_batched_f16
+#define mi355det_sgd_pack_step mi355det_sgd_pack_step_f16
+#define mi355det_sgd_pack_table_build mi355det_sgd_pack_table_build_f16
+#define mi355det_sgd_pack_table_bytes mi355det_sgd_pack_table_bytes_f16
 #define mi355det_stem_im2col mi355det_stem_im2col_f16
 #define mi355det_unpack_wgrad mi355det_unpack_wgrad_f16
 #define mi355det_conv_wgrad mi355det_conv_wgrad_f16
@@ -53,4 +56,5 @@
 #define g_wgrad_ablate g_wgrad_ablate_f16
 #define g_dgrad_s2_off g_dgrad_s2_off_f16
 #define pack_batched_kernel pack_batched_kernel_f16
+#define sgd_pack_kernel sgd_pack_kernel_f16
 #define splitk_reduce_kernel splitk_reduce_kernel_f16
diff --git a/object_detectors_amd/csrc/sgd_update.h b/object_detectors_amd/csrc/sgd_update.h
--- /dev/null
+++ b/object_detectors_amd/csrc/sgd_update.h
@@ -0,0 +1,16 @@
+#pragma once
+#include <hip/hip_runtime.h>
+
+struct SgdArgs {
+  float lr, momentum, dampening, wd, gscale;
+  int nesterov, first, zero_grad;
+};
+
+__device__ __forceinline__ void sgd_update(float& w, float g, float& m, const SgdArgs& a) {
+  float d = __fmaf_rn(g, a.gscale, __fmul_rn(a.wd, w));
+  if (a.momentum != 0.f) {
+    m = a.first ? d : __fmaf_rn(1.f - a.dampening, d, __fmul_rn(a.momentum, m));
+    d = a.nesterov ? __fmaf_rn(a.momentum, m, d) : m;
+  }
+  w = __fmaf_rn(-a.lr, d, w);
+}
diff --git a/object_detectors_amd/optim.py b/object_detectors_amd/optim.py
--- a/object_detectors_amd/optim.py
+++ b/object_detectors_amd/optim.py
@@ -1,3 +1,5 @@
+import os
+
 import torch
 
 from ._lib import check, lib
@@ -16,10 +18,17 @@
         self.flat_w, self.flat_g = flat_w, flat_g
         super().__init__([flat_w], defaults)
         self.steps = 0
+        self.engine = None
 
     @classmethod
     def for_engine(cls, engine, **kw):
-        return cls(engine.flat_w, engine.flat_g, **kw)
+        opt = cls(engine.flat_w, engine.flat_g, **kw)
+        opt.engine = engine
+        return opt
+
+    def _masters_changed(self):
+        if getattr(self.engine, "packs_current", None) is not None:
+            self.engine.packs_current = None
 
     def zero_grad(self, set_to_none=False):
         self.flat_g.zero_()
@@ -30,17 +39,29 @@
     def __init__(self, flat_w, flat_g, lr=1e-3, momentum=0.0, dampening=0.0, weight_decay=0.0, nesterov=False):
         super().__init__(flat_w, flat_g, dict(lr=lr, momentum=momentum, dampening=dampening, weight_decay=weight_decay, nesterov=nesterov))
         self.momentum_buf = torch.zeros_like(flat_w)
+        self.fused = False
+
+    @classmethod
+    def for_engine(cls, engine, **kw):
+        opt = super().for_engine(engine, **kw)
+        opt.fused = os.environ.get("MI355DET_FUSED_STEP", "1") != "0" and hasattr(engine, "packs_current")
+        return opt
 
     @torch.no_grad()
     def step(self, closure=None, grad_scale=1.0, zero_grad=False, skip_flag=None):
         g = self.param_groups[0]
-        st = lib().mi355det_sgd_step_guarded(self.flat_w.data_ptr(), self.flat_g.data_ptr(), self.momentum_buf.data_ptr(), self.flat_w.numel(),
-                                             float(g["lr"]), float(g["momentum"]), float(g["dampening"]), float(g["weight_decay"]),
-                                             float(grad_scale), int(bool(g["nesterov"])), int(self.steps == 0), int(zero_grad),
-                                             None if skip_flag is None else skip_flag.data_ptr(), _stream())
-        check(st, "sgd_step")
+        bufs = (self.flat_w.data_ptr(), self.flat_g.data_ptr(), self.momentum_buf.data_ptr())
+        args = (float(g["lr"]), float(g["momentum"]), float(g["dampening"]), float(g["weight_decay"]), float(grad_scale),
+                int(bool(g["nesterov"])), int(self.steps == 0), int(zero_grad), None if skip_flag is None else skip_flag.data_ptr(), _stream())
+        plan = getattr(self.engine, "_last_plan", None) if self.fused else None
+        if plan is not None and plan.training:
+            tab, ne, nb = plan.step_table()
+            check(plan.L.mi355det_sgd_pack_step(tab.data_ptr(), ne, nb, *bufs, *args), "sgd_pack_step")
+            self.engine.packs_current = plan
+        else:
+            self._masters_changed()
+            check(lib().mi355det_sgd_step_guarded(*bufs, self.flat_w.numel(), *args), "sgd_step")
         self.steps += 1
-
 
     def reference_state_dict(self, engine):
         g = self.param_groups[0]
@@ -76,6 +97,7 @@
     def step(self, closure=None, grad_scale=1.0, zero_grad=False, skip_flag=None):
         g = self.param_groups[0]
         self.steps += 1
+        self._masters_changed()
         st = lib().mi355det_adam_step_guarded(self.flat_w.data_ptr(), self.flat_g.data_ptr(), self.exp_avg.data_ptr(), self.exp_avg_sq.data_ptr(),
                                               self.flat_w.numel(), float(g["lr"]), float(g["betas"][0]), float(g["betas"][1]), float(g["eps"]),
                                               float(g["weight_decay"]), float(grad_scale), self.steps, int(zero_grad),
diff --git a/object_detectors_amd/plan_core.py b/object_detectors_amd/plan_core.py
--- a/object_detectors_amd/plan_core.py
+++ b/object_detectors_amd/plan_core.py
@@ -60,7 +60,7 @@
     return p
 
 
-def build_pack_table(L, eng, specs, shape_of, need_dgrad):
+def build_pack_table(L, eng, specs, shape_of, need_dgrad, step=False):
     items = (_lib.PackItem * max(1, len(specs)))()
     for i, s in enumerate(specs):
         wf, wd = eng.packed[s.name]
@@ -70,9 +70,11 @@
         items[i].shape, items[i].cout_pad = shape_of(s)
         items[i].w_is_ohwi = 1
     ne, nb = C.c_int32(0), C.c_int32(0)
-    nbytes = L.mi355det_pack_table_bytes(items, len(specs), C.byref(ne), C.byref(nb))
+    flat = (_vp(eng.flat_w), eng.flat_w.numel()) if step else ()
+    size, build = (L.mi355det_sgd_pack_table_bytes, L.mi355det_sgd_pack_table_build) if step else (L.mi355det_pack_table_bytes, L.mi355det_pack_table_build)
+    nbytes = size(items, len(specs), *flat, C.byref(ne), C.byref(nb))
     host = torch.empty(max(nbytes, 1), dtype=torch.uint8)
-    check(L.mi355det_pack_table_build(items, len(specs), C.c_void_p(host.data_ptr()), nbytes), "pack_table_build")
+    check(build(items, len(specs), *flat, C.c_void_p(host.data_ptr()), nbytes), "sgd_pack_table_build" if step else "pack_table_build")
     return host.to(eng.device), ne.value, nb.value
 
 
@@ -99,6 +101,13 @@
     def build_pack_table(self, specs, shape_of, need_dgrad):
         self.pack_table, ne, nb = build_pack_table(self.L, self.eng, specs, shape_of, need_dgrad)
         self.pack.append((self.L.mi355det_pack_weights_batched, (_vp(self.pack_table), ne, nb, self.stream)))
+        self._pack_args = (specs, shape_of, need_dgrad)
+        self._step_table = None
+
+    def step_table(self):
+        if self._step_table is None:
+            self._step_table = build_pack_table(self.L, self.eng, *self._pack_args, step=True)
+        return self._step_table
 
     @contextlib.contextmanager
     def autotuning(self):
diff --git a/object_detectors_amd/yolo/nets/engine.py b/object_detectors_amd/yolo/nets/engine.py
--- a/object_detectors_amd/yolo/nets/engine.py
+++ b/object_detectors_amd/yolo/nets/engine.py
@@ -79,6 +79,7 @@
         self.head_ld = ops.pad_to(self.head_c, 32)
         self._static_epoch = 1
         self._frozen = False
+        self.packs_current = None
         self.specs = arch(backbone, num_anchors, num_classes)
         self.by_name = {s.name: s for s in self.specs}
         self._layout_params()
@@ -90,9 +91,11 @@
     def freeze_inference(self, on=True):
         self._static_epoch += 1
         self._frozen = bool(on)
+        self.packs_current = None
 
     def _weights_changed(self):
         self._static_epoch += 1
+        self.packs_current = None
 
     def _layout_params(self):
         off = 0
@@ -624,8 +627,10 @@
         self._set_image(images)
         eng = self.eng
         if self.training:
+            packed = eng.packs_current is self
             eng._weights_changed()
-            self._run(self.pack)
+            if not packed:
+                self._run(self.pack)
         elif not (eng._frozen and self._const_epoch == eng._static_epoch):
             self._run(self.pack)
             self._run(self.fwd_const)
```
